# FudanCVL/SynFMC

Hardware: AMD Instinct MI355X
Metric: denoising steps/sec, 16x320x512 bf16 U-Net+CMC+OMC (higher is better)
Workload: dtype bf16; 1 GPU; 16x320x512 clip, CFG batch 2, full-width 3D U-Net (1.39B params, random init) + Camera Adapter (CMC) + Object Motion Control (OMC) features, DDIM step; configs/obj.yaml shapes; 1 clip per GPU; frames=16, height=320, width=512, hip_graph=True, fp8_temporal_attention=False, parallelism=dp1 (independent clips, no collective)

## Files before the change

include/fmc_hip.h:

```cpp
#ifndef FMC_HIP_H
#define FMC_HIP_H

#include <stdint.h>

#ifdef __cplusplus
extern "C" {
#endif

#define FMC_VERSION 100

enum { FMC_BF16 = 0, FMC_F32 = 1 };

enum {
    FMC_OK = 0,
    FMC_E_SHAPE = -1,
    FMC_E_DTYPE = -2,
    FMC_E_ALIGN = -3,
    FMC_E_LAUNCH = -4,
    FMC_E_NULL = -5
};

int fmc_version(void);
const char* fmc_last_error(void);

int64_t fmc_groupnorm_workspace_bytes(int N, int C, int G);
int fmc_groupnorm_silu_fwd(const void* x, void* y, const float* gamma, const float* beta, float* stats,
                           void* workspace, int N, int HW, int C, int G, float eps, int act, int dtype,
                           const void* x2, int C1, void* stream);
int fmc_groupnorm_silu_bwd(const void* dy, const void* x, void* dx, const float* gamma, const float* beta,
                           const float* stats, void* workspace, int N, int HW, int C, int G, int act,
                           int dtype, void* stream);

int fmc_layernorm_fwd(const void* x, void* y, const float* gamma, const float* beta, const float* pe,
                      int64_t M, int C, float eps, int pe_inner, int pe_frames, int dtype, void* stream);
int fmc_layernorm_add_fwd(const void* x, const void* addend, void* sum_out, void* y, const float* gamma, const float* beta,
                          const float* pe, int64_t M, int C, float eps, int pe_inner, int pe_frames, int dtype, void* stream);

int fmc_geglu_fwd(const void* x, void* y, int64_t M, int Cff, int dtype, void* stream);

int fmc_spatial_attn_fwd(const void* q, const void* k, const void* v, void* o, float* lse, int B, int H,
                         int Sq, int Skv, int D, int64_t q_batch_stride, int64_t q_row_stride,
                         int64_t kv_batch_stride, int64_t kv_row_stride, int64_t o_batch_stride,
                         int64_t o_row_stride, int kv_batch_div, float scale, int dtype, void* stream);

int fmc_temporal_attn_fwd(const void* q, const void* k, const void* v, void* o, int n_clips, int n_pix,
                          int F, int H, int D, int64_t clip_stride, int64_t frame_stride,
                          int64_t pix_stride, int64_t o_clip_stride, int64_t o_frame_stride,
                          int64_t o_pix_stride, float scale, int dtype, void* stream);

int fmc_plucker_fwd(const float* K, const float* c2w, void* out, int B, int F, int H, int W, int c2w_rows,
                    int layout, int dtype, void* stream);

int fmc_omc_rasterize_fwd(const float* poses, const float* masks, void* feat, float* mask_out, int BF,
                          int n_obj, int H, int W, int layout, int dtype, void* stream);

int fmc_gaussian_circle_mask_fwd(const float* circles, float* out, int N, int H, int W, void* stream);

int fmc_mask_modulate_fwd(const void* x, const float* mask_in, void* y, float* mask_out, int N, int h, int w,
                          int C, int Hin, int Win, int dtype, void* stream);

int fmc_feature_add_fwd(const void* h, const void* t, void* out, int64_t n_elems, int64_t skip_elems,
                        int dtype, void* stream);

int fmc_cfg_ddim_step(const void* eps_uc, const float* x, float* x_out, int64_t n, int has_uncond,
                      float guidance, float alpha_t, float alpha_prev, int dtype, void* stream);

typedef struct fmc_sampler_coef {
    float g;
    float m_x, m_e, m_clamp;
    float c_x, c_e, c_m, c_n;
    float c_h[3];
    float in_scale;
} fmc_sampler_coef;
int64_t fmc_sampler_step_elems_per_trip(void);
int fmc_sampler_step(const void* eps_uc, const float* x, const void* noise, const float* hist0, const float* hist1,
                     const float* hist2, float* x_out, float* m_out, void* x_in, int64_t n, int has_uncond, int n_hist,
                     int in_reps, fmc_sampler_coef coef, int dtype, int in_dtype, void* stream);

int fmc_linear_bf16(const void* x, const void* w, const void* bias, const void* residual, void* out, int64_t M, int N,
                    int K, int64_t ldx, int64_t ldres, int64_t ldo, float alpha, int epilogue, int tile, int split_k,
                    void* workspace, int64_t workspace_bytes, const void* x2, int64_t ldx2, int k_split,
                    const void* residual2, void* stream);

int fmc_conv3x3_bf16(const void* x, const void* w, const void* bias, const void* temb, const void* residual, void* out,
                     int n_img, int H, int W, int Cin, int Cout, int64_t temb_row_stride, int temb_img_div,
                     int upsample2x, int tile, int split_k, void* workspace, int64_t workspace_bytes, void* stream);

int fmc_linear_bf16_gn(const void* x, const void* w, const void* bias, const void* residual, void* out, int64_t M, int N, int K,
                       int64_t ldx, int64_t ldres, int64_t ldo, float alpha, const void* residual2, float* gn_partials, int gn_hw,
                       int w_tilemajor, void* stream);
int fmc_linear_bf16_ln(const void* x, const void* w, const void* bias, const void* residual, void* out, int64_t M, int N, int K,
                       int64_t ldx, int64_t ldres, int64_t ldo, float alpha, const void* residual2, void* ln_out, const float* ln_gamma,
                       const float* ln_beta, float ln_eps, const float* ln_pe, int ln_pe_inner, int ln_pe_frames, float* ln_stats, int w_tilemajor,
                       void* stream);
int fmc_linear_bf16_lnc(const void* x, const void* w_gamma, void* out, int64_t M, int N, int K, int64_t ldx, int64_t ldo, int epilogue,
                        const float* ln_stats, const float* ln_c, const float* ln_bias, int w_tilemajor, void* stream);
int fmc_linear_bf16_ffblk(const void* x, const void* w, const void* bias, const void* residual, void* out, int64_t M, int N, int K,
                          int64_t ldres, float alpha, int epilogue, int x_blocked, int out_blocked, const float* ln_stats, const float* ln_c,
                          const float* ln_bias, int w_tilemajor, void* stream);
int fmc_groupnorm_fold_linear(const float* partials, int part_splits, const float* gamma, const float* beta, const void* w, const void* bias,
                              void* w_out, float* bias_out, int n_img, int HW, int C, int G, int N, float eps, int w_tilemajor, void* stream);
int fmc_linear_bf16_imgw(const void* x, const void* w_img, const float* bias_img, void* out, int64_t M, int N, int K, int64_t ldx, int64_t ldo,
                         int img_rows, float* ln_stats, float ln_eps, int w_tilemajor, void* stream);
int fmc_linear_bf16_fftail(const void* x_blocked, const void* x2, const void* w, const void* bias, const void* residual, void* out, int64_t M,
                           int N, int K, int k_split, int64_t ldx2, int64_t ldres, float* gn_partials, int gn_hw, int w_tilemajor, void* stream);
int fmc_linear_bf16_ffblk_partial(const void* x_blocked, const void* w, const void* bias, const void* residual, void* out, int64_t M, int N, int K,
                                  int64_t ldres, float alpha, int w_tilemajor, void* stream);
int fmc_linear_bf16_fftail_partial(const void* x_blocked, const void* x2, const void* w, const void* bias, const void* residual, void* out, int64_t M,
                                   int N, int K, int k_split, int64_t ldx2, int64_t ldres, float* gn_partials, int gn_hw, int w_tilemajor, void* stream);
int fmc_conv3x3_bf16_gn(const void* x, const void* w, const void* bias, const void* temb, const void* residual, void* out, int n_img,
                        int H, int W, int Cin, int Cout, int64_t temb_row_stride, int temb_img_div, int upsample2x,
                        float* gn_partials, int w_tilemajor, void* stream);
int fmc_groupnorm_apply_fwd(const void* x, void* y, const float* gamma, const float* beta, float* stats, const float* partials,
                            int part_splits, int N, int HW, int C, int G, float eps, int act, int dtype, void* stream);

int fmc_linear4_supported(int64_t M, int N, int K, int64_t ldx);
int fmc_linear4_bf16(const void* x, const void* w, const void* bias, const void* residual, const void* residual2, void* out, int64_t M, int N, int K,
                     int64_t ldx, int64_t ldres, int64_t ldo, float alpha, void* stream);

int fmc_vendor_init(void);
int fmc_vendor_destroy(void);
int fmc_vendor_version(void);
int64_t fmc_vendor_workspace_bytes(void);
int fmc_vendor_linear_candidates(int64_t M, int N, int K, int64_t ldx, int64_t ldres, int64_t ldo, int has_bias, int has_residual);
int fmc_vendor_linear_bf16(const void* x, const void* w, const void* bias, const void* residual, void* out, int64_t M, int N, int K,
                           int64_t ldx, int64_t ldres, int64_t ldo, int algo, void* workspace, int64_t workspace_bytes, void* stream);

int fmc_attention_supported(int D);
int fmc_attention_fwd(const void* q, const void* k, const void* v, void* o, const unsigned char* key_keep, int B, int H, int Sq, int Skv, int D,
                      int64_t q_batch_stride, int64_t q_row_stride, int64_t kv_batch_stride, int64_t kv_row_stride, int64_t o_batch_stride,
                      int64_t o_row_stride, float scale, int causal, int dtype, void* stream);

int fmc_geglu_pipe_supported(int64_t M, int cff, int C, int variant);
int fmc_geglu_pipe_ln_bf16(const void* h, void* out, const float* ln_gamma, const float* ln_beta, float ln_eps, const void* w_packed, const void* bias,
                           int64_t M, int cff, int C, int out_blocked, int variant, void* stream);
int fmc_geglu_pipe_partial_supported(int64_t M, int cff, int C, int variant);
int fmc_geglu_pipe_ln_partial_bf16(const void* h, void* out, const float* ln_gamma, const float* ln_beta, float ln_eps, const void* w_packed, const void* bias,
                                   int64_t M, int cff, int C, int out_blocked, int variant, void* stream);

int fmc_groupnorm_partial_splits(int HW, int C);
int fmc_groupnorm_partials(const void* x, const void* x2, int C1, float* partials, int N, int HW, int C, int G, int dtype, void* stream);
int fmc_conv3x3_halo_supported(int n_img, int H, int W, int Cin, int Cin1, int Cout, int upsample2x);
int64_t fmc_conv3x3_halo_packed_bytes(int Cin, int Cout);
int fmc_conv3x3_halo_pack_weight(const void* w, void* dst, int Cin, int Cout, void* stream);
int fmc_conv3x3_halo_tiles_per_image(int H, int W);
int fmc_conv3x3_halo_bf16(const void* x, const void* x2, int Cin1, const void* w_packed, const void* bias, const void* temb, const void* residual,
                          void* out, int n_img, int H, int W, int Cin, int Cout, int64_t temb_row_stride, int temb_img_div, int upsample2x,
                          const float* gn_coef, int gn_act, float* gn_partials, void* stream);
int fmc_conv3x3_halo_sc_supported(int n_img, int H, int W, int Cin, int Cout, int Cin_sc, int Cin_sc1);
int64_t fmc_conv3x3_halo_sc_packed_bytes(int Cin, int Cout, int Cin_sc);
int64_t fmc_conv3x3_halo_sc_pack_source(int64_t chunk, int Cin, int Cin_sc, int tile_channels, int* from_shortcut);
int fmc_conv3x3_halo_sc_pack_weight(const void* w, const void* w_sc, void* dst, int Cin, int Cout, int Cin_sc, int tile_channels, void* stream);
int fmc_conv3x3_halo_sc_bf16(const void* x, const void* w_packed, const void* bias, const void* temb, void* out, const void* xs, const void* xs2,
                             int Cin_sc1, int Cin_sc, int n_img, int H, int W, int Cin, int Cout, int64_t temb_row_stride, int temb_img_div,
                             float* gn_partials, void* stream);
int fmc_conv3x3_halo4_supported(int n_img, int H, int W, int Cin, int Cin1, int Cout, int upsample2x, int wide);
int fmc_conv3x3_halo4_pack_weight(const void* w, void* dst, int Cin, int Cout, int wide, void* stream);
int fmc_conv3x3_halo4_row_blocks_per_image(int H, int W);
int fmc_conv3x3_halo4_tiles(int n_img, int H, int W, int Cout, int wide);
int fmc_conv3x3_halo4_bf16(const void* x, const void* x2, int Cin1, const void* w_packed, const void* bias, const void* temb, const void* residual,
                           void* out, int n_img, int H, int W, int Cin, int Cout, int64_t temb_row_stride, int temb_img_div, int upsample2x,
                           float* gn_partials, int split_k, void* workspace, int64_t workspace_bytes, int wide, void* stream);
int64_t fmc_conv3x3_upfold_packed_bytes(int Cin, int Cout);
int fmc_conv3x3_upfold_pack_weight(const void* w, void* dst, int Cin, int Cout, int tile_channels, void* stream);
int fmc_conv3x3_halo_fold_supported(int n_img, int Hs, int Ws, int Cin, int Cout);
int fmc_conv3x3_halo_fold_bf16(const void* x, const void* w_folded, const void* bias, void* out, int n_img, int Hs, int Ws, int Cin, int Cout,
                               float* gn_partials, void* stream);
int fmc_conv3x3_halo4_fold_supported(int n_img, int Hs, int Ws, int Cin, int Cout, int wide);
int fmc_conv3x3_halo4_fold_bf16(const void* x, const void* w_folded, const void* bias, void* out, int n_img, int Hs, int Ws, int Cin, int Cout,
                                float* gn_partials, int wide, void* stream);
int fmc_conv3x3_halo_partial_supported(int n_img, int H, int W, int Cin, int Cin1, int Cout, int upsample2x);
int fmc_conv3x3_halo_partial_tiles_per_image(int H, int W);
int fmc_conv3x3_halo_partial_bf16(const void* x, const void* x2, int Cin1, const void* w_packed, const void* bias, const void* temb,
                                  const void* residual, void* out, int n_img, int H, int W, int Cin, int Cout, int64_t temb_row_stride,
                                  int temb_img_div, int upsample2x, const float* gn_coef, int gn_act, float* gn_partials, void* stream);
int fmc_conv3x3_halo_sc_partial_supported(int n_img, int H, int W, int Cin, int Cout, int Cin_sc, int Cin_sc1);
int fmc_conv3x3_halo_sc_partial_bf16(const void* x, const void* w_packed, const void* bias, const void* temb, void* out, const void* xs,
                                     const void* xs2, int Cin_sc1, int Cin_sc, int n_img, int H, int W, int Cin, int Cout, int64_t temb_row_stride,
                                     int temb_img_div, float* gn_partials, void* stream);
int fmc_conv3x3_halo_fold_partial_supported(int n_img, int Hs, int Ws, int Cin, int Cout);
int fmc_conv3x3_halo_fold_partial_bf16(const void* x, const void* w_folded, const void* bias, void* out, int n_img, int Hs, int Ws, int Cin,
                                       int Cout, float* gn_partials, void* stream);
int fmc_conv3x3_halo4_partial_supported(int n_img, int H, int W, int Cin, int Cin1, int Cout, int upsample2x, int wide);
int fmc_conv3x3_halo4_partial_tw(int H, int W, int wide);
int fmc_conv3x3_halo4_partial_row_blocks_per_image(int H, int W, int tw);
int fmc_conv3x3_halo4_partial_tiles(int n_img, int H, int W, int Cout, int wide, int tw);
int fmc_conv3x3_halo4_partial_bf16(const void* x, const void* x2, int Cin1, const void* w_packed, const void* bias, const void* temb,
                                   const void* residual, void* out, int n_img, int H, int W, int Cin, int Cout, int64_t temb_row_stride,
                                   int temb_img_div, int upsample2x, float* gn_partials, int split_k, void* workspace, int64_t workspace_bytes,
                                   int wide, int tw, void* stream);
int fmc_conv3x3_halo4_fold_partial_supported(int n_img, int Hs, int Ws, int Cin, int Cout, int wide);
int fmc_conv3x3_halo4_fold_partial_bf16(const void* x, const void* w_folded, const void* bias, void* out, int n_img, int Hs, int Ws, int Cin,
                                        int Cout, float* gn_partials, int wide, int tw, void* stream);
int fmc_conv3x3_down_bwd_supported(int n_img, int H, int W, int Cin, int Cout);
int64_t fmc_conv3x3_down_bwd_packed_bytes(int Cin, int Cout);
int fmc_conv3x3_down_bwd_pack_weight(const void* w, void* dst, int Cin, int Cout, void* stream);
int fmc_conv3x3_down_bwd_tile(int n_img, int H, int W, int Cin, int Cout);
int fmc_conv3x3_down_bwd_bf16(const void* dy, const void* w_packed, void* dx, int n_img, int H, int W, int Cin, int Cout, int tile, void* stream);
int fmc_conv3x3_up_bwd_supported(int n_img, int Hs, int Ws, int Cin, int Cout);
int64_t fmc_conv3x3_up_bwd_packed_bytes(int Cin, int Cout);
int fmc_conv3x3_up_bwd_pack_weight(const void* w, void* dst, int Cin, int Cout, void* stream);
int fmc_conv3x3_up_bwd_tile(int n_img, int Hs, int Ws, int Cin, int Cout);
int fmc_conv3x3_up_bwd_bf16(const void* dy, const void* w_packed, void* dx, int n_img, int Hs, int Ws, int Cin, int Cout, int tile, void* stream);
int fmc_groupnorm_coef(const float* partials, int part_splits, const float* gamma, const float* beta, float* coef, float* stats, int N, int HW,
                       int C, int G, float eps, void* stream);

int fmc_split_bf16x3(const float* src, void* dst, int64_t rows, int C, int64_t ld_src, int64_t ld_dst, int col0, int K,
                     int role, void* stream);
int fmc_linear_x3_f32(const void* x3, const void* w3, const float* bias, const float* residual, float* out, int64_t M, int N,
                      int K3, int64_t ldx, int64_t ldres, int64_t ldo, float alpha, int epilogue, int tile, int split_k,
                      void* workspace, int64_t workspace_bytes, const float* residual2, void* stream);
int fmc_conv3x3_x3_f32(const void* x3, const void* w3, const float* bias, const float* temb, const float* residual, float* out,
                       int n_img, int H, int W, int Cin3, int Cout, int64_t temb_row_stride, int temb_img_div,
                       int upsample2x, int tile, int split_k, void* workspace, int64_t workspace_bytes, void* stream);

int fmc_layernorm_bwd(const void* dy, const void* x, const float* gamma, void* dx, float* dgamma, float* dbeta,
                      int64_t M, int C, float eps, int dtype, void* stream);
int fmc_layernorm_bwd_add(const void* dy, const void* x, const float* gamma, void* dx, float* dgamma, float* dbeta, const void* addend,
                          int64_t M, int C, float eps, int dtype, void* stream);
int fmc_groupnorm_silu_bwd_add(const void* dy, const void* x, void* dx, const float* gamma, const float* beta, const float* stats,
                               void* workspace, int N, int HW, int C, int G, int act, const void* addend, int dtype, void* stream);
int64_t fmc_groupnorm_silu_bwd_params_workspace_bytes(int N, int HW, int C, int G);
int fmc_groupnorm_silu_bwd_params(const void* dy, const void* x, void* dx, float* dgamma, float* dbeta, const float* gamma,
                                  const float* beta, const float* stats, const void* addend, int accumulate, void* workspace,
                                  int N, int HW, int C, int G, int act, int dtype, void* stream);
int64_t fmc_column_sum_workspace_bytes(int64_t M, int N);
int fmc_column_sum(const void* x, float* out, int64_t M, int N, int64_t ld, float alpha, int accumulate, void* workspace, int dtype,
                   void* stream);
int fmc_geglu_bwd(const void* dy, const void* x, void* dx, int64_t M, int Cff, int dtype, void* stream);
int fmc_spatial_attn_bwd(const void* q, const void* k, const void* v, const void* o, const void* d_o, const float* lse,
                         float* dvec, void* dq, void* dk, void* dv, int B, int H, int Sq, int Skv, int D,
                         int64_t q_batch_stride, int64_t q_row_stride, int64_t kv_batch_stride, int64_t kv_row_stride,
                         int64_t o_batch_stride, int64_t o_row_stride, int64_t dq_batch_stride, int64_t dq_row_stride,
                         int64_t dkv_batch_stride, int64_t dkv_row_stride, int kv_batch_div, float scale, int dtype,
                         void* stream);
int fmc_temporal_attn_bwd(const void* q, const void* k, const void* v, const void* d_o, void* dq, void* dk, void* dv,
                          int n_clips, int n_pix, int F, int H, int D, int64_t clip_stride, int64_t frame_stride,
                          int64_t pix_stride, int64_t do_clip_stride, int64_t do_frame_stride, int64_t do_pix_stride,
                          int64_t dq_clip_stride, int64_t dq_frame_stride, int64_t dq_pix_stride, float scale,
                          int dtype, void* stream);

int fmc_fp8_scales_roll(void* amax, void* scale, void* inv_scale, float margin, void* stream);
int fmc_linear_fp8_qkv(const void* x, const void* w, void* out_fp8, int64_t M, int N, int K, int64_t ldx,
                       const void* inv_scales, void* amax_bits, void* stream);
int fmc_temporal_attn_fp8_fwd(const void* q, const void* k, const void* v, void* o, const void* scales, int n_clips,
                              int n_pix, int F, int H, int D, int64_t clip_stride, int64_t frame_stride,
                              int64_t pix_stride, int64_t o_clip_stride, int64_t o_frame_stride, int64_t o_pix_stride,
                              float scale, void* stream);
int fmc_temporal_attn_fp8_bwd(const void* q, const void* k, const void* v, const void* scales, const void* d_o, void* dq,
                              void* dk, void* dv, int n_clips, int n_pix, int F, int H, int D, int64_t clip_stride,
                              int64_t frame_stride, int64_t pix_stride, int64_t do_clip_stride, int64_t do_frame_stride,
                              int64_t do_pix_stride, int64_t dq_clip_stride, int64_t dq_frame_stride,
                              int64_t dq_pix_stride, float scale, void* stream);

int fmc_nhwc_to_cmajor_padded(const void* src, void* dst, int n_img, int H, int W, int C, int64_t row_len, int guard,
                              int shifts, void* stream);
// ... 96 lines not shown
```

synfmc_amd/_lib.py:

```python
from __future__ import annotations

import ctypes
import os
from ctypes import c_char_p, c_float, c_int, c_int64, c_void_p

_HERE = os.path.dirname(os.path.abspath(__file__))
LIB_PATH = os.environ.get("FMC_HIP_LIB") or os.path.join(_HERE, "lib", "libfmc_hip.so")

FMC_BF16, FMC_F32 = 0, 1

_ERRORS = {-1: ValueError, -2: TypeError, -3: ValueError, -4: RuntimeError, -5: ValueError}


class SamplerCoef(ctypes.Structure):
    _fields_ = [("g", c_float), ("m_x", c_float), ("m_e", c_float), ("m_clamp", c_float), ("c_x", c_float), ("c_e", c_float),
                ("c_m", c_float), ("c_n", c_float), ("c_h", c_float * 3), ("in_scale", c_float)]

SIGNATURES = {
    "fmc_version": (c_int, []),
    "fmc_last_error": (c_char_p, []),
    "fmc_groupnorm_workspace_bytes": (c_int64, [c_int, c_int, c_int]),
    "fmc_groupnorm_silu_fwd": (c_int, [c_void_p, c_void_p, c_void_p, c_void_p, c_void_p, c_void_p, c_int, c_int, c_int,
                                       c_int, c_float, c_int, c_int, c_void_p, c_int, c_void_p]),
    "fmc_groupnorm_silu_bwd": (c_int, [c_void_p, c_void_p, c_void_p, c_void_p, c_void_p, c_void_p, c_void_p, c_int,
                                       c_int, c_int, c_int, c_int, c_int, c_void_p]),
    "fmc_layernorm_add_fwd": (c_int, [c_void_p, c_void_p, c_void_p, c_void_p, c_void_p, c_void_p, c_void_p, c_int64, c_int, c_float, c_int,
                                      c_int, c_int, c_void_p]),
    "fmc_layernorm_fwd": (c_int, [c_void_p, c_void_p, c_void_p, c_void_p, c_void_p, c_int64, c_int, c_float, c_int,
                                  c_int, c_int, c_void_p]),
    "fmc_geglu_fwd": (c_int, [c_void_p, c_void_p, c_int64, c_int, c_int, c_void_p]),
    "fmc_spatial_attn_fwd": (c_int, [c_void_p, c_void_p, c_void_p, c_void_p, c_void_p, c_int, c_int, c_int, c_int, c_int,
                                     c_int64, c_int64, c_int64, c_int64, c_int64, c_int64, c_int, c_float, c_int,
                                     c_void_p]),
    "fmc_temporal_attn_fwd": (c_int, [c_void_p, c_void_p, c_void_p, c_void_p, c_int, c_int, c_int, c_int, c_int,
                                      c_int64, c_int64, c_int64, c_int64, c_int64, c_int64, c_float, c_int, c_void_p]),
    "fmc_plucker_fwd": (c_int, [c_void_p, c_void_p, c_void_p, c_int, c_int, c_int, c_int, c_int, c_int, c_int, c_void_p]),
    "fmc_omc_rasterize_fwd": (c_int, [c_void_p, c_void_p, c_void_p, c_void_p, c_int, c_int, c_int, c_int, c_int, c_int,
                                      c_void_p]),
    "fmc_gaussian_circle_mask_fwd": (c_int, [c_void_p, c_void_p, c_int, c_int, c_int, c_void_p]),
    "fmc_mask_modulate_fwd": (c_int, [c_void_p, c_void_p, c_void_p, c_void_p, c_int, c_int, c_int, c_int, c_int, c_int,
                                      c_int, c_void_p]),
    "fmc_feature_add_fwd": (c_int, [c_void_p, c_void_p, c_void_p, c_int64, c_int64, c_int, c_void_p]),
    "fmc_cfg_ddim_step": (c_int, [c_void_p, c_void_p, c_void_p, c_int64, c_int, c_float, c_float, c_float, c_int,
                                  c_void_p]),
    "fmc_sampler_step_elems_per_trip": (c_int64, []),
    "fmc_sampler_step": (c_int, [c_void_p] * 9 + [c_int64, c_int, c_int, c_int, SamplerCoef, c_int, c_int, c_void_p]),
    "fmc_linear_bf16": (c_int, [c_void_p, c_void_p, c_void_p, c_void_p, c_void_p, c_int64, c_int, c_int, c_int64,
                                c_int64, c_int64, c_float, c_int, c_int, c_int, c_void_p, c_int64, c_void_p, c_int64, c_int,
                                c_void_p, c_void_p]),
    "fmc_linear_bf16_gn": (c_int, [c_void_p, c_void_p, c_void_p, c_void_p, c_void_p, c_int64, c_int, c_int, c_int64, c_int64, c_int64,
                                   c_float, c_void_p, c_void_p, c_int, c_int, c_void_p]),
    "fmc_linear_bf16_ln": (c_int, [c_void_p, c_void_p, c_void_p, c_void_p, c_void_p, c_int64, c_int, c_int, c_int64, c_int64, c_int64,
                                   c_float, c_void_p, c_void_p, c_void_p, c_void_p, c_float, c_void_p, c_int, c_int, c_void_p, c_int, c_void_p]),
    "fmc_linear_bf16_lnc": (c_int, [c_void_p, c_void_p, c_void_p, c_int64, c_int, c_int, c_int64, c_int64, c_int, c_void_p, c_void_p, c_void_p,
                                    c_int, c_void_p]),
    "fmc_linear_bf16_ffblk": (c_int, [c_void_p, c_void_p, c_void_p, c_void_p, c_void_p, c_int64, c_int, c_int, c_int64, c_float, c_int, c_int, c_int,
                                      c_void_p, c_void_p, c_void_p, c_int, c_void_p]),
    "fmc_groupnorm_fold_linear": (c_int, [c_void_p, c_int, c_void_p, c_void_p, c_void_p, c_void_p, c_void_p, c_void_p, c_int, c_int, c_int, c_int, c_int,
                                          c_float, c_int, c_void_p]),
    "fmc_linear_bf16_imgw": (c_int, [c_void_p, c_void_p, c_void_p, c_void_p, c_int64, c_int, c_int, c_int64, c_int64, c_int, c_void_p, c_float, c_int,
                                     c_void_p]),
    "fmc_linear_bf16_fftail": (c_int, [c_void_p, c_void_p, c_void_p, c_void_p, c_void_p, c_void_p, c_int64, c_int, c_int, c_int, c_int64, c_int64,
                                       c_void_p, c_int, c_int, c_void_p]),
    "fmc_conv3x3_bf16_gn": (c_int, [c_void_p, c_void_p, c_void_p, c_void_p, c_void_p, c_void_p, c_int, c_int, c_int, c_int, c_int,
                                    c_int64, c_int, c_int, c_void_p, c_int, c_void_p]),
    "fmc_groupnorm_partial_splits": (c_int, [c_int, c_int]),
    "fmc_groupnorm_partials": (c_int, [c_void_p, c_void_p, c_int, c_void_p, c_int, c_int, c_int, c_int, c_int, c_void_p]),
    "fmc_conv3x3_halo_supported": (c_int, [c_int, c_int, c_int, c_int, c_int, c_int, c_int]),
    "fmc_conv3x3_halo_packed_bytes": (c_int64, [c_int, c_int]),
    "fmc_conv3x3_halo_pack_weight": (c_int, [c_void_p, c_void_p, c_int, c_int, c_void_p]),
    "fmc_conv3x3_halo_tiles_per_image": (c_int, [c_int, c_int]),
    "fmc_conv3x3_halo_sc_supported": (c_int, [c_int, c_int, c_int, c_int, c_int, c_int, c_int]),
    "fmc_conv3x3_halo_sc_packed_bytes": (c_int64, [c_int, c_int, c_int]),
    "fmc_conv3x3_halo_sc_pack_source": (c_int64, [c_int64, c_int, c_int, c_int, ctypes.POINTER(c_int)]),
    "fmc_conv3x3_halo_sc_pack_weight": (c_int, [c_void_p, c_void_p, c_void_p, c_int, c_int, c_int, c_int, c_void_p]),
    "fmc_conv3x3_halo_sc_bf16": (c_int, [c_void_p, c_void_p, c_void_p, c_void_p, c_void_p, c_void_p, c_void_p, c_int, c_int, c_int, c_int, c_int,
                                         c_int, c_int, c_int64, c_int, c_void_p, c_void_p]),
    "fmc_conv3x3_halo_bf16": (c_int, [c_void_p, c_void_p, c_int, c_void_p, c_void_p, c_void_p, c_void_p, c_void_p, c_int, c_int, c_int, c_int, c_int,
                                      c_int64, c_int, c_int, c_void_p, c_int, c_void_p, c_void_p]),
    "fmc_conv3x3_halo4_supported": (c_int, [c_int, c_int, c_int, c_int, c_int, c_int, c_int, c_int]),
    "fmc_conv3x3_halo4_pack_weight": (c_int, [c_void_p, c_void_p, c_int, c_int, c_int, c_void_p]),
    "fmc_conv3x3_halo4_row_blocks_per_image": (c_int, [c_int, c_int]),
    "fmc_conv3x3_halo4_tiles": (c_int, [c_int, c_int, c_int, c_int, c_int]),
    "fmc_conv3x3_halo4_bf16": (c_int, [c_void_p, c_void_p, c_int, c_void_p, c_void_p, c_void_p, c_void_p, c_void_p, c_int, c_int, c_int, c_int, c_int,
                                       c_int64, c_int, c_int, c_void_p, c_int, c_void_p, c_int64, c_int, c_void_p]),
    "fmc_conv3x3_upfold_packed_bytes": (c_int64, [c_int, c_int]),
    "fmc_conv3x3_upfold_pack_weight": (c_int, [c_void_p, c_void_p, c_int, c_int, c_int, c_void_p]),
    "fmc_conv3x3_halo_fold_supported": (c_int, [c_int, c_int, c_int, c_int, c_int]),
    "fmc_conv3x3_halo_fold_bf16": (c_int, [c_void_p, c_void_p, c_void_p, c_void_p, c_int, c_int, c_int, c_int, c_int, c_void_p, c_void_p]),
    "fmc_conv3x3_halo4_fold_supported": (c_int, [c_int, c_int, c_int, c_int, c_int, c_int]),
    "fmc_conv3x3_halo4_fold_bf16": (c_int, [c_void_p, c_void_p, c_void_p, c_void_p, c_int, c_int, c_int, c_int, c_int, c_void_p, c_int, c_void_p]),
    "fmc_conv3x3_halo_partial_supported": (c_int, [c_int, c_int, c_int, c_int, c_int, c_int, c_int]),
    "fmc_conv3x3_halo_partial_tiles_per_image": (c_int, [c_int, c_int]),
    "fmc_conv3x3_halo_partial_bf16": (c_int, [c_void_p, c_void_p, c_int, c_void_p, c_void_p, c_void_p, c_void_p, c_void_p, c_int, c_int, c_int, c_int,
                                              c_int, c_int64, c_int, c_int, c_void_p, c_int, c_void_p, c_void_p]),
    "fmc_conv3x3_halo_sc_partial_supported": (c_int, [c_int, c_int, c_int, c_int, c_int, c_int, c_int]),
    "fmc_conv3x3_halo_sc_partial_bf16": (c_int, [c_void_p, c_void_p, c_void_p, c_void_p, c_void_p, c_void_p, c_void_p, c_int, c_int, c_int, c_int,
                                                 c_int, c_int, c_int, c_int64, c_int, c_void_p, c_void_p]),
    "fmc_conv3x3_halo_fold_partial_supported": (c_int, [c_int, c_int, c_int, c_int, c_int]),
    "fmc_conv3x3_halo_fold_partial_bf16": (c_int, [c_void_p, c_void_p, c_void_p, c_void_p, c_int, c_int, c_int, c_int, c_int, c_void_p, c_void_p]),
    "fmc_conv3x3_halo4_partial_supported": (c_int, [c_int, c_int, c_int, c_int, c_int, c_int, c_int, c_int]),
    "fmc_conv3x3_halo4_partial_tw": (c_int, [c_int, c_int, c_int]),
    "fmc_conv3x3_halo4_partial_row_blocks_per_image": (c_int, [c_int, c_int, c_int]),
    "fmc_conv3x3_halo4_partial_tiles": (c_int, [c_int, c_int, c_int, c_int, c_int, c_int]),
    "fmc_conv3x3_halo4_partial_bf16": (c_int, [c_void_p, c_void_p, c_int, c_void_p, c_void_p, c_void_p, c_void_p, c_void_p, c_int, c_int, c_int, c_int,
                                               c_int, c_int64, c_int, c_int, c_void_p, c_int, c_void_p, c_int64, c_int, c_int, c_void_p]),
    "fmc_conv3x3_halo4_fold_partial_supported": (c_int, [c_int, c_int, c_int, c_int, c_int, c_int]),
    "fmc_conv3x3_halo4_fold_partial_bf16": (c_int, [c_void_p, c_void_p, c_void_p, c_void_p, c_int, c_int, c_int, c_int, c_int, c_void_p, c_int, c_int,
                                                    c_void_p]),
    "fmc_conv3x3_down_bwd_supported": (c_int, [c_int, c_int, c_int, c_int, c_int]),
    "fmc_conv3x3_down_bwd_packed_bytes": (c_int64, [c_int, c_int]),
    "fmc_conv3x3_down_bwd_pack_weight": (c_int, [c_void_p, c_void_p, c_int, c_int, c_void_p]),
    "fmc_conv3x3_down_bwd_tile": (c_int, [c_int, c_int, c_int, c_int, c_int]),
    "fmc_conv3x3_down_bwd_bf16": (c_int, [c_void_p, c_void_p, c_void_p, c_int, c_int, c_int, c_int, c_int, c_int, c_void_p]),
    "fmc_conv3x3_up_bwd_supported": (c_int, [c_int, c_int, c_int, c_int, c_int]),
    "fmc_conv3x3_up_bwd_packed_bytes": (c_int64, [c_int, c_int]),
    "fmc_conv3x3_up_bwd_pack_weight": (c_int, [c_void_p, c_void_p, c_int, c_int, c_void_p]),
    "fmc_conv3x3_up_bwd_tile": (c_int, [c_int, c_int, c_int, c_int, c_int]),
    "fmc_conv3x3_up_bwd_bf16": (c_int, [c_void_p, c_void_p, c_void_p, c_int, c_int, c_int, c_int, c_int, c_int, c_void_p]),
    "fmc_linear4_supported": (c_int, [c_int64, c_int, c_int, c_int64]),
    "fmc_vendor_linear_candidates": (c_int, [c_int64, c_int, c_int, c_int64, c_int64, c_int64, c_int, c_int]),
    "fmc_vendor_linear_bf16": (c_int, [c_void_p, c_void_p, c_void_p, c_void_p, c_void_p, c_int64, c_int, c_int, c_int64, c_int64, c_int64, c_int, c_void_p,
                                       c_int64, c_void_p]),
    "fmc_geglu_pipe_supported": (c_int, [c_int64, c_int, c_int, c_int]),
    "fmc_geglu_pipe_ln_bf16": (c_int, [c_void_p, c_void_p, c_void_p, c_void_p, c_float, c_void_p, c_void_p, c_int64, c_int, c_int, c_int, c_int, c_void_p]),
    "fmc_geglu_pipe_partial_supported": (c_int, [c_int64, c_int, c_int, c_int]),
    "fmc_geglu_pipe_ln_partial_bf16": (c_int, [c_void_p, c_void_p, c_void_p, c_void_p, c_float, c_void_p, c_void_p, c_int64, c_int, c_int, c_int, c_int,
                                               c_void_p]),
    "fmc_linear_bf16_ffblk_partial": (c_int, [c_void_p, c_void_p, c_void_p, c_void_p, c_void_p, c_int64, c_int, c_int, c_int64, c_float, c_int, c_void_p]),
    "fmc_linear_bf16_fftail_partial": (c_int, [c_void_p, c_void_p, c_void_p, c_void_p, c_void_p, c_void_p, c_int64, c_int, c_int, c_int, c_int64, c_int64,
                                               c_void_p, c_int, c_int, c_void_p]),
    "fmc_attention_supported": (c_int, [c_int]),
    "fmc_attention_fwd": (c_int, [c_void_p, c_void_p, c_void_p, c_void_p, c_void_p, c_int, c_int, c_int, c_int, c_int, c_int64, c_int64, c_int64, c_int64,
                                  c_int64, c_int64, c_float, c_int, c_int, c_void_p]),
    "fmc_vendor_init": (c_int, []),
    "fmc_vendor_destroy": (c_int, []),
    "fmc_vendor_version": (c_int, []),
    "fmc_vendor_workspace_bytes": (c_int64, []),
    "fmc_linear4_bf16": (c_int, [c_void_p, c_void_p, c_void_p, c_void_p, c_void_p, c_void_p, c_int64, c_int, c_int, c_int64, c_int64, c_int64, c_float, c_void_p]),
    "fmc_groupnorm_coef": (c_int, [c_void_p, c_int, c_void_p, c_void_p, c_void_p, c_void_p, c_int, c_int, c_int, c_int, c_float, c_void_p]),
    "fmc_groupnorm_apply_fwd": (c_int, [c_void_p, c_void_p, c_void_p, c_void_p, c_void_p, c_void_p, c_int, c_int, c_int, c_int, c_int,
                                        c_float, c_int, c_int, c_void_p]),
    "fmc_split_bf16x3": (c_int, [c_void_p, c_void_p, c_int64, c_int, c_int64, c_int64, c_int, c_int, c_int, c_void_p]),
    "fmc_linear_x3_f32": (c_int, [c_void_p, c_void_p, c_void_p, c_void_p, c_void_p, c_int64, c_int, c_int, c_int64,
                                  c_int64, c_int64, c_float, c_int, c_int, c_int, c_void_p, c_int64, c_void_p, c_void_p]),
    "fmc_conv3x3_x3_f32": (c_int, [c_void_p, c_void_p, c_void_p, c_void_p, c_void_p, c_void_p, c_int, c_int, c_int,
                                   c_int, c_int, c_int64, c_int, c_int, c_int, c_int, c_void_p, c_int64, c_void_p]),
    "fmc_layernorm_bwd": (c_int, [c_void_p, c_void_p, c_void_p, c_void_p, c_void_p, c_void_p, c_int64, c_int, c_float,
                                  c_int, c_void_p]),
    "fmc_layernorm_bwd_add": (c_int, [c_void_p, c_void_p, c_void_p, c_void_p, c_void_p, c_void_p, c_void_p, c_int64, c_int, c_float,
                                      c_int, c_void_p]),
    "fmc_groupnorm_silu_bwd_add": (c_int, [c_void_p, c_void_p, c_void_p, c_void_p, c_void_p, c_void_p, c_void_p, c_int, c_int, c_int, c_int,
                                           c_int, c_void_p, c_int, c_void_p]),
    "fmc_groupnorm_silu_bwd_params_workspace_bytes": (c_int64, [c_int, c_int, c_int, c_int]),
    "fmc_groupnorm_silu_bwd_params": (c_int, [c_void_p] * 9 + [c_int, c_void_p] + [c_int] * 6 + [c_void_p]),
    "fmc_column_sum_workspace_bytes": (c_int64, [c_int64, c_int]),
    "fmc_column_sum": (c_int, [c_void_p, c_void_p, c_int64, c_int, c_int64, c_float, c_int, c_void_p, c_int, c_void_p]),
    "fmc_geglu_bwd": (c_int, [c_void_p, c_void_p, c_void_p, c_int64, c_int, c_int, c_void_p]),
    "fmc_spatial_attn_bwd": (c_int, [c_void_p] * 10 + [c_int] * 5 + [c_int64] * 10 + [c_int, c_float, c_int, c_void_p]),
    "fmc_temporal_attn_bwd": (c_int, [c_void_p] * 7 + [c_int] * 5 + [c_int64] * 9 + [c_float, c_int, c_void_p]),
    "fmc_fp8_scales_roll": (c_int, [c_void_p, c_void_p, c_void_p, c_float, c_void_p]),
    "fmc_linear_fp8_qkv": (c_int, [c_void_p, c_void_p, c_void_p, c_int64, c_int, c_int, c_int64, c_void_p, c_void_p, c_void_p]),
    "fmc_temporal_attn_fp8_fwd": (c_int, [c_void_p] * 5 + [c_int] * 5 + [c_int64] * 6 + [c_float, c_void_p]),
    "fmc_temporal_attn_fp8_bwd": (c_int, [c_void_p] * 8 + [c_int] * 5 + [c_int64] * 9 + [c_float, c_void_p]),
    "fmc_nhwc_to_cmajor_padded": (c_int, [c_void_p, c_void_p, c_int, c_int, c_int, c_int, c_int64, c_int, c_int, c_void_p]),
    "fmc_linear_wgrad_workspace_bytes": (c_int64, [c_void_p, c_int]),
    "fmc_linear_wgrad_bf16": (c_int, [c_void_p, c_int, c_void_p, c_int64, c_void_p]),
    "fmc_conv3x3_wgrad_supported": (c_int, [c_int, c_int, c_int, c_int, c_int, c_int]),
    "fmc_conv3x3_wgrad_workspace_bytes": (c_int64, [c_int, c_int, c_int, c_int, c_int, c_int]),
    "fmc_conv3x3_wgrad_bf16": (c_int, [c_void_p, c_void_p, c_void_p, c_int, c_int, c_int, c_int, c_int, c_int, c_int, c_float, c_int, c_void_p,
                               c_int64, c_void_p]),
    "fmc_optim_chunk_elems": (c_int, []),
    "fmc_optim_workspace_bytes": (c_int64, [c_int, c_int, c_int]),
    "fmc_optim_check_tables": (c_int, [c_void_p, c_int, c_void_p, c_int, c_int, c_int]),
    "fmc_optim_grad_norm": (c_int, [c_void_p, c_int, c_void_p, c_int, c_void_p, c_int, c_int, c_void_p, c_int64, c_void_p]),
    "fmc_optim_adamw_step": (c_int, [c_void_p, c_int, c_void_p, c_int, c_void_p, c_int, c_int, c_void_p, c_int64, c_void_p]),
    "fmc_avgpool2x2_fwd": (c_int, [c_void_p, c_void_p, c_int, c_int, c_int, c_int, c_void_p]),
    "fmc_avgpool2x2_bwd": (c_int, [c_void_p, c_void_p, c_int, c_int, c_int, c_int, c_void_p]),
    "fmc_relu_fwd": (c_int, [c_void_p, c_void_p, c_int64, c_void_p]),
    "fmc_relu_bwd": (c_int, [c_void_p, c_void_p, c_void_p, c_int64, c_void_p]),
    "fmc_add_bf16": (c_int, [c_void_p, c_void_p, c_void_p, c_int64, c_void_p]),
    "fmc_temporal_block_bf16": (c_int, [c_void_p, c_void_p, c_void_p, c_void_p, c_float, c_void_p, c_void_p, c_float, c_void_p, c_void_p, c_void_p,
                                        c_void_p, c_float, c_int, c_int, c_int, c_int, c_int, c_float, c_void_p]),
    "fmc_temporal_block_set_debug": (c_int, [c_void_p]),
    "fmc_xattn_block640_bf16": (c_int, [c_void_p, c_void_p, c_void_p, c_void_p, c_float, c_void_p, c_void_p, c_void_p, c_void_p, c_int, c_int, c_int, c_int,
                                        c_float, c_void_p]),
    "fmc_xattn_pack_kv": (c_int, [c_void_p, c_void_p, c_int, c_int, c_int64, c_void_p]),
    "fmc_geglu320_ln_bf16": (c_int, [c_void_p, c_void_p, c_void_p, c_void_p, c_float, c_void_p, c_void_p, c_int64, c_int, c_int, c_void_p]),
    "fmc_geglu640_ln_bf16": (c_int, [c_void_p, c_void_p, c_void_p, c_void_p, c_float, c_void_p, c_void_p, c_int64, c_int, c_int, c_void_p]),
    "fmc_xattn_pack_kv40": (c_int, [c_void_p, c_void_p, c_int, c_int, c_int64, c_void_p]),
    "fmc_xattn_block320_bf16": (c_int, [c_void_p, c_void_p, c_void_p, c_void_p, c_float, c_void_p, c_void_p, c_void_p, c_void_p, c_void_p, c_float,
                                        c_int, c_int, c_int, c_int, c_float, c_void_p]),
    "fmc_temporal_block_partial_bf16": (c_int, [c_void_p, c_void_p, c_void_p, c_void_p, c_float, c_void_p, c_void_p, c_float, c_void_p, c_void_p, c_void_p,
                                                c_void_p, c_float, c_int, c_int, c_int, c_int, c_int, c_float, c_void_p]),
    "fmc_xattn_block640_partial_bf16": (c_int, [c_void_p, c_void_p, c_void_p, c_void_p, c_float, c_void_p, c_void_p, c_void_p, c_void_p, c_int, c_int, c_int,
                                                c_int, c_float, c_void_p]),
    "fmc_xattn_block320_partial_bf16": (c_int, [c_void_p, c_void_p, c_void_p, c_void_p, c_float, c_void_p, c_void_p, c_void_p, c_void_p, c_void_p, c_float,
                                                c_int, c_int, c_int, c_int, c_float, c_void_p]),
    "fmc_mxfp8_tile_rows": (c_int, []),
    "fmc_mxfp8_tile_cols": (c_int, []),
    "fmc_linear_mxfp8_supported": (c_int, [c_int64, c_int, c_int, c_int]),
    "fmc_mxfp8_pack_weight": (c_int, [c_void_p, c_void_p, c_void_p, c_int, c_int, c_int, c_void_p]),
    "fmc_layernorm_mxfp8_fwd": (c_int, [c_void_p, c_void_p, c_void_p, c_void_p, c_void_p, c_int64, c_int, c_int64, c_float, c_void_p]),
    "fmc_linear_mxfp8": (c_int, [c_void_p, c_void_p, c_void_p, c_void_p, c_void_p, c_void_p, c_void_p, c_void_p, c_int64, c_int, c_int, c_int64, c_int64,
                                 c_int, c_void_p]),
    "fmc_conv3x3_bf16": (c_int,[c_void_p, c_void_p, c_void_p, c_void_p, c_void_p, c_void_p, c_int, c_int, c_int,
                                 c_int, c_int, c_int64, c_int, c_int, c_int, c_int, c_void_p, c_int64, c_void_p]),
}

_lib = None


class FmcLibraryMissing(ImportError):
    pass
# ... 24 lines not shown
```

synfmc_amd/csrc/gemm_conv.hip:

```cpp
#include <stdlib.h>

#include <algorithm>
#include <type_traits>

#include "common.h"

namespace {

constexpr int BK_MAX = 64;

struct GemmParams {
    const bf16_t* a; const bf16_t* w; const bf16_t* bias; const bf16_t* temb; const bf16_t* res; bf16_t* out;
    const bf16_t* res2;
    int64_t M; int N, K;
    int64_t lda, ldres, ldo;
    int img_h, img_w, cin, hw;
    int64_t temb_ld; int temb_div;
    const bf16_t* a2; int64_t lda2; int ksplit;
    int ups;
    float alpha;
    int tiles_m, tiles_n;
    int regepi;
    int tap_outer;
    int group_m;
// ... 2096 lines not shown
    auto up4 = [](const bf16_t* p, float (&o)[4]) {
        const u32x2 w = *reinterpret_cast<const u32x2*>(p);
        o[0] = __uint_as_float(w[0] << 16); o[1] = __uint_as_float(w[0] & 0xffff0000u);
        o[2] = __uint_as_float(w[1] << 16); o[3] = __uint_as_float(w[1] & 0xffff0000u);
    };
    float o[4] = {v[0], v[1], v[2], v[3]}, a[4];
    if (P.bias) {
        up4(P.bias + n, a);
#pragma unroll
        for (int j = 0; j < 4; ++j) o[j] += a[j];
    }
#pragma unroll
    for (int j = 0; j < 4; ++j) o[j] *= P.alpha;
    if (MODE == 1 && P.temb) {
        up4(P.temb + ((m / P.hw) / P.temb_div) * P.temb_ld + n, a);
#pragma unroll
        for (int j = 0; j < 4; ++j) o[j] += a[j];
    }
    if (P.res) {
        up4(P.res + m * P.ldres + n, a);
#pragma unroll
        for (int j = 0; j < 4; ++j) o[j] += a[j];
        if (P.res2) {
            up4(P.res2 + m * P.ldres + n, a);
#pragma unroll
            for (int j = 0; j < 4; ++j) o[j] += a[j];
        }
    }
    *reinterpret_cast<u32x2*>(P.out + m * P.ldo + n) = u32x2{pack_bf2(o[0], o[1]), pack_bf2(o[2], o[3])};
}

template <int MODE, int EPI, int WM, int WN, int BK, int STAGES, int MI = 2>
void launch_gemm_g(GemmParams& P, hipStream_t st) {
    constexpr int BM = 32 * MI * WM, BN = 64 * WN;
    P.tiles_m = (int)((P.M + BM - 1) / BM);
    P.tiles_n = (P.N + BN - 1) / BN;
    P.tap_outer = conv_tap_outer();
    static const int regepi = fmc_env_int("FMC_GEMM_REGEPI", 1);
    P.regepi = regepi;
    size_t lds = (size_t)STAGES * (BM + BN) * BK * sizeof(bf16_t) + 1024;
    const size_t slab = (size_t)64 * (BN + 8) * sizeof(float);
    if (slab > lds) lds = slab;
    const size_t staged = (size_t)BM * ((EPI == 1 ? BN / 2 : BN) + 8) * sizeof(bf16_t);
    const size_t lds_plain = (P.split_k == 1 && (EPI == 1 || !P.res2) && staged > lds) ? staged : lds;
    unsigned grid = (unsigned)(P.tiles_m * P.tiles_n * P.split_k);
    constexpr int by_waves = 16 / (WM * WN) > 0 ? 16 / (WM * WN) : 1;
    const int by_lds = (int)(160 * 1024 / (P.sk ? lds : lds_plain));
    const int per_cu = by_lds < by_waves ? (by_lds < 1 ? 1 : by_lds) : by_waves;
    P.group_m = xcd_group_m(P, MODE == 0, 32.0 * per_cu, BN, BM);
    if (P.sk) {
        const int64_t iters = (int64_t)P.tiles_m * P.tiles_n * (P.K / BK);
        const int g = (fmc_cu_count() * per_cu) & ~7;
        const int64_t need = (int64_t)g * BM * BN * (int64_t)sizeof(float) + 4096;
        if (STAGES != 2 || MI != 2 || g < 8 || iters < 4 * (int64_t)g || P.sk_ws_bytes < need || g * (int)sizeof(int) > 4096) {
            P.sk = 0;
        } else {
            P.sk = g;
            grid = (unsigned)g;
        }
    }
    if constexpr (STAGES == 2 && MI == 2) {
        if (P.sk) {
            fmc_launch<gemm_kernel<MODE, EPI, WM, WN, MI, BK, STAGES, true>>(dim3(grid), dim3(64 * WM * WN), lds, st, P);
            return;
        }
    }
    fmc_launch<gemm_kernel<MODE, EPI, WM, WN, MI, BK, STAGES, false>>(dim3(grid), dim3(64 * WM * WN), lds_plain, st, P);
    if (P.split_k > 1) {
        const int64_t chunks = P.M * (P.N / 8);
        hipLaunchKernelGGL(splitk_reduce_kernel, dim3((unsigned)((chunks + 255) / 256)), dim3(256), 0, st, P);
    }
}

template <int MODE, int EPI, int PF>
void launch_gemm8(GemmParams& P, hipStream_t st) {
    P.tiles_m = (int)((P.M + 255) / 256);
    P.tiles_n = (P.N + 255) / 256;
    P.tap_outer = conv_tap_outer();
    P.group_m = xcd_group_m(P, MODE == 0, 32.0, 1, 1);
    constexpr size_t ring = (size_t)2 * 512 * 64 * sizeof(bf16_t) + 1024;
    constexpr size_t staged = (size_t)256 * ((EPI != 0 ? 128 : 256) + 8) * sizeof(bf16_t);
    constexpr size_t lds = staged > ring ? staged : ring;
    constexpr auto plain = gemm8_kernel<MODE, EPI, PF, 0>, sk_main = gemm8_kernel<MODE, EPI, PF, 1>, sk_finish = gemm8_kernel<MODE, EPI, PF, 2>;
    const int tiles = P.tiles_m * P.tiles_n;
    P.sk_t0 = 0;
    if (P.sk && P.sk_hybrid && !P.sk_lock) {
        const int g = fmc_cu_count() & ~7;
        const int t0 = g >= 8 ? (tiles / g) * g : 0, rem = tiles - t0;
        const int64_t iters = (int64_t)rem * (P.K / 64);
        const int maxseg = (rem + g - 1) / (g > 0 ? g : 1) + 2;
        const int64_t need = (int64_t)g * maxseg * 256 * 256 * (int64_t)sizeof(float) + 4096;
        if (t0 > 0 && rem > 0 && iters >= 2 * (int64_t)g && P.sk_ws_bytes >= need && need < ((int64_t)1 << 31)) {
            P.sk = g;
            P.sk_maxseg = maxseg;
            P.sk_whole = 0;
            P.sk_t0 = t0;
            fmc_launch<sk_main>(dim3((unsigned)g), dim3(512), lds, st, P);
            fmc_launch<plain>(dim3((unsigned)t0), dim3(512), lds, st, P);
            fmc_launch<sk_finish>(dim3((unsigned)rem), dim3(512), lds, st, P);
            return;
        }
        if (rem == 0) P.sk = 0;
    }
    if (P.sk && P.sk_lock) {
        const int g = fmc_cu_count() & ~7, nkt = P.K / 64;
        int S = P.sk_lock > 1 ? P.sk_lock : 0;
        if (!S) {
            double best = 1e30;
            for (int s2 = 2; s2 <= 16 && s2 <= nkt / 4; ++s2) {
                const int L = (nkt + s2 - 1) / s2;
                if ((s2 - 1) * L >= nkt) continue;
                const int rounds = (tiles * s2 + g - 1) / (g > 0 ? g : 1);
                const double cost = rounds * (L * 1.9 + 4.0) + tiles * s2 * 0.06;
                if (cost < best) { best = cost; S = s2; }
            }
        }
        const int L = S ? (nkt + S - 1) / S : 0;
        const int64_t need = (int64_t)tiles * S * 256 * 256 * (int64_t)sizeof(float) + 4096;
        if (g >= 8 && S >= 2 && (S - 1) * L < nkt && P.sk_ws_bytes >= need && need < ((int64_t)1 << 31)) {
            P.sk = g;
            P.sk_lock = S;
            P.sk_lock_len = L;
            fmc_launch<sk_main>(dim3((unsigned)g), dim3(512), lds, st, P);
            if constexpr (EPI == 0) hipLaunchKernelGGL((sk_finish_kernel<MODE>), dim3((unsigned)tiles * 64), dim3(256), 0, st, P);
            else fmc_launch<sk_finish>(dim3((unsigned)tiles), dim3(512), lds, st, P);
            return;
        }
        P.sk_lock = 0;
    }
    if (P.sk) {
        const int64_t iters = (int64_t)tiles * (P.K / 64);
        const int g = fmc_cu_count() & ~7;
        const int maxseg = (tiles + g - 1) / g + 2;
        const int64_t need = (int64_t)g * maxseg * 256 * 256 * (int64_t)sizeof(float) + 4096;
        if (g >= 8 && iters >= 2 * (int64_t)g && P.sk_ws_bytes >= need && need < ((int64_t)1 << 31)) {
            P.sk = g;
            P.sk_maxseg = maxseg;
            P.sk_whole = 0;
            fmc_launch<sk_main>(dim3((unsigned)g), dim3(512), lds, st, P);
            fmc_launch<sk_finish>(dim3((unsigned)tiles), dim3(512), lds, st, P);
            return;
        }
        P.sk = 0;
    }
    fmc_launch<plain>(dim3((unsigned)tiles), dim3(512), lds, st, P);
}

constexpr int K320_K = 320;
template <int MI, int NI> constexpr int k320_stage_chunks() { return ((32 * MI * ((160 * NI + 8) / 8) + 63) / 64) * 64; }
template <int MI, int NI> constexpr size_t k320_lds() {
    return (size_t)2 * 32 * MI * K320_K * 2 + (size_t)k320_stage_chunks<MI, NI>() * 16 + 160 * NI * sizeof(float);
}

template <int MI, int NI, bool HAS_RES>
__global__ __launch_bounds__(320, (MI * NI == 1 ? 3 : (MI * NI == 2 ? 2 : 1))) void gemm_k320_kernel(const GemmParams P) {
    constexpr int K = K320_K, KS = K / 16, BM = 32 * MI, BN = 160 * NI, OP = BN + 8, CPR = K / 8, OCPR = OP / 8, WC = 32 * NI;
    constexpr int A_ELEMS = BM * K, A_PIECES = BM * CPR / 64, ST_PIECES = k320_stage_chunks<MI, NI>() / 64;
    constexpr int A_PPW = (A_PIECES + 4) / 5, ST_PPW = (ST_PIECES + 4) / 5;
    extern __shared__ __attribute__((aligned(16))) unsigned char smem_raw[];
    bf16_t* Abuf = reinterpret_cast<bf16_t*>(smem_raw);
    bf16_t* Os = Abuf + 2 * A_ELEMS;
    float* bias_s = reinterpret_cast<float*>(Os + k320_stage_chunks<MI, NI>() * 8);
    const int tid = threadIdx.x, lane = tid & 63, wave = __builtin_amdgcn_readfirstlane(tid >> 6);
    const int l31 = lane & 31, half = lane >> 5;
    const int n0 = blockIdx.y * BN;
    const int ntiles = (int)(P.M / BM);

    bf16x8 wf[KS][NI];
#pragma unroll
    for (int ni = 0; ni < NI; ++ni) {
        const bf16_t* wrow = P.w + (int64_t)(n0 + wave * WC + ni * 32 + l31) * K + half * 8;
#pragma unroll
        for (int ks = 0; ks < KS; ++ks) {
            union { bf16x8 v; u32x4 u; } t;
            t.u = *reinterpret_cast<const u32x4*>(wrow + ks * 16);
            wf[ks][ni] = t.v;
        }
    }
    for (int i = tid; i < BN; i += 320) bias_s[i] = P.bias ? bf2f(P.bias[n0 + i]) : 0.f;

    const __amdgpu_buffer_rsrc_t rsA = __builtin_amdgcn_make_buffer_rsrc((void*)P.a, 0, (int)(((P.M - 1) * P.lda + K) * 2), 0x00020000);
    const __amdgpu_buffer_rsrc_t rsR = __builtin_amdgcn_make_buffer_rsrc((void*)(HAS_RES ? P.res + n0 : P.a), 0,
                                                                         HAS_RES ? (int)(((P.M - 1) * P.ldres + BN) * 2) : 0, 0x00020000);
    constexpr unsigned OOB = 0x7ffffff0u;
    int lane_v = lane, tid_v = tid;
    auto a_vo = [&](int piece) {
        const int L = piece * 64 + lane_v, row = L / CPR, phys = L - row * CPR;
        return (unsigned)(row * (int)P.lda * 2 + (phys ^ ((row >> 1) & 7)) * 16);
    };
    auto r_vo = [&](int piece) {
        const int L = piece * 64 + lane_v, row = L / OCPR, cc = L - row * OCPR;
        return (row < BM && cc < BN / 8) ? (unsigned)(row * (int)P.ldres * 2 + cc * 16) : OOB;
    };
    auto dma = [&](const __amdgpu_buffer_rsrc_t& rs, unsigned voff, int soff, bf16_t* lds) {
        __builtin_amdgcn_raw_ptr_buffer_load_lds(rs, (__attribute__((address_space(3))) void*)lds, 16, (int)voff, soff, 0, 0);
    };
    auto load_a = [&](int tile, int buf) {
        const int soff = tile * BM * (int)P.lda * 2;
#pragma unroll
        for (int i = 0; i < A_PPW; ++i)
            if (wave + 5 * i < A_PIECES) dma(rsA, a_vo(wave + 5 * i), soff, Abuf + buf * A_ELEMS + (wave + 5 * i) * 512);
    };
    auto load_res = [&](int tile) {
        const int soff = tile * BM * (int)P.ldres * 2;
#pragma unroll
        for (int i = 0; i < ST_PPW; ++i)
            if (wave + 5 * i < ST_PIECES) dma(rsR, r_vo(wave + 5 * i), soff, Os + (wave + 5 * i) * 512);
    };

    const int sw = (l31 >> 1) & 7, x6 = sw & 6, b0 = half ^ (sw & 1);
    int dsel[4];
#pragma unroll
    for (int m = 0; m < 4; ++m) dsel[m] = l31 * K + (x6 - 2 * (x6 & (2 * m)) + b0) * 8;

    int t = blockIdx.x;
    if (t < ntiles) load_a(t, 0);
    if (t + (int)gridDim.x < ntiles) load_a(t + gridDim.x, 1);
    if (HAS_RES && t < ntiles) load_res(t);
    asm volatile("s_waitcnt vmcnt(0)" ::: "memory");
    __syncthreads();

    for (int it = 0; t < ntiles; t += gridDim.x, ++it) {
        const bf16_t* As = Abuf + (it & 1) * A_ELEMS;
        asm volatile("" : "+v"(lane_v), "+v"(tid_v));
        f32x16 acc[NI][MI];
#pragma unroll
        for (int a = 0; a < NI; ++a)
#pragma unroll
            for (int g = 0; g < 4; ++g) {
                const f32x4 bv = *reinterpret_cast<const f32x4*>(bias_s + wave * WC + a * 32 + 8 * g + 4 * half);
#pragma unroll
                for (int b = 0; b < MI; ++b)
#pragma unroll
                    for (int j = 0; j < 4; ++j) acc[a][b][4 * g + j] = bv[j];
            }
        bf16x8 af[2][MI];
        auto read_a = [&](int ks, bf16x8 (&f)[MI]) {
#pragma unroll
            for (int mi = 0; mi < MI; ++mi) {
                union { bf16x8 v; u32x4 u; } ta;
                ta.u = *reinterpret_cast<const u32x4*>(As + mi * 32 * K + dsel[ks & 3] + ks * 16);
                f[mi] = ta.v;
            }
        };
        read_a(0, af[0]);
#pragma unroll
        for (int ks = 0; ks < KS; ++ks) {
            if (ks + 1 < KS) read_a(ks + 1, af[(ks + 1) & 1]);
            __builtin_amdgcn_sched_barrier(0);
#pragma unroll
            for (int ni = 0; ni < NI; ++ni)
#pragma unroll
                for (int mi = 0; mi < MI; ++mi)
                    acc[ni][mi] = __builtin_amdgcn_mfma_f32_32x32x16_bf16(wf[ks][ni], af[ks & 1][mi], acc[ni][mi], 0, 0, 0);
            __builtin_amdgcn_sched_barrier(0);
        }
        asm volatile("s_waitcnt vmcnt(0) lgkmcnt(0)\n\ts_barrier" ::: "memory");
        asm volatile("" : "+v"(lane_v), "+v"(tid_v));
        const int l31_e = lane_v & 31, half_e = (lane_v >> 5) & 1;
        if (t + 2 * (int)gridDim.x < ntiles) load_a(t + 2 * gridDim.x, it & 1);

#pragma unroll
        for (int ni = 0; ni < NI; ++ni)
#pragma unroll
            for (int mi = 0; mi < MI; ++mi) {
                bf16_t* wbase = Os + (mi * 32 + l31_e) * OP + wave * WC + ni * 32 + 4 * half_e;
                u32x2 rw[4];
                if (HAS_RES) {
#pragma unroll
                    for (int g = 0; g < 4; ++g) rw[g] = *reinterpret_cast<const u32x2*>(wbase + 8 * g);
                }
#pragma unroll
                for (int g = 0; g < 4; ++g) {
                    float o[4];
#pragma unroll
                    for (int j = 0; j < 4; ++j) o[j] = P.alpha * acc[ni][mi][4 * g + j];
                    if (HAS_RES) {
                        o[0] += __uint_as_float(rw[g][0] << 16); o[1] += __uint_as_float(rw[g][0] & 0xffff0000u);
                        o[2] += __uint_as_float(rw[g][1] << 16); o[3] += __uint_as_float(rw[g][1] & 0xffff0000u);
                    }
                    *reinterpret_cast<u32x2*>(wbase + 8 * g) = u32x2{pack_bf2(o[0], o[1]), pack_bf2(o[2], o[3])};
                }
            }
        asm volatile("s_waitcnt lgkmcnt(0)\n\ts_barrier" ::: "memory");
        {
            bf16_t* og = P.out + (int64_t)t * BM * P.ldo + n0;
            for (int c = tid_v; c < BM * (BN / 8); c += 320) {
                const int r = c / (BN / 8), ch = c - r * (BN / 8);
                *reinterpret_cast<u32x4*>(og + (int64_t)r * P.ldo + ch * 8) = *reinterpret_cast<const u32x4*>(Os + r * OP + ch * 8);
            }
        }
        if (HAS_RES) {
            asm volatile("s_waitcnt lgkmcnt(0)\n\ts_barrier" ::: "memory");
            if (t + (int)gridDim.x < ntiles) load_res(t + gridDim.x);
        }
    }
}

inline int gemm_k320_cfg() {
    static const int v = fmc_env_int("FMC_K320_CFG", 22);
    return v;
}
bool gemm_k320_ok(const GemmParams& P) {
    const int bn = (gemm_k320_cfg() % 10 == 1) ? 160 : 320;
    return !P.f32io && P.hw <= 1 && P.K == K320_K && P.N % bn == 0 && P.M % 64 == 0 && !P.a2 && !P.res2 && P.split_k == 1 && !P.sk && !P.temb &&
           ((P.M - 1) * P.lda + P.K) * 2 < ((int64_t)1 << 31) && (!P.res || ((P.M - 1) * P.ldres + P.N) * 2 < ((int64_t)1 << 31));
}

template <int MI, int NI>
void launch_gemm_k320_c(GemmParams& P, hipStream_t st) {
    const size_t lds = k320_lds<MI, NI>();
    const int per_cu = MI * NI == 1 ? 3 : (MI * NI == 2 ? 2 : 1);
    const int tiles = (int)(P.M / (32 * MI)), slots = fmc_cu_count() * per_cu;
    dim3 grid((unsigned)(tiles < slots ? tiles : slots), (unsigned)(P.N / (160 * NI)));
    if (P.res) fmc_launch<gemm_k320_kernel<MI, NI, true>>(grid, dim3(320), lds, st, P);
    else fmc_launch<gemm_k320_kernel<MI, NI, false>>(grid, dim3(320), lds, st, P);
}
void launch_gemm_k320(GemmParams& P, hipStream_t st) {
    switch (gemm_k320_cfg()) {
        case 11: launch_gemm_k320_c<1, 1>(P, st); break;
        case 21: launch_gemm_k320_c<2, 1>(P, st); break;
        case 12: launch_gemm_k320_c<1, 2>(P, st); break;
        default: launch_gemm_k320_c<2, 2>(P, st); break;
    }
}

bool gemm160_ok(const GemmParams& P) {
    return P.N % 320 == 0 && !P.sk && (!P.a2 || P.a_blocked);
}
template <int MODE, int EPI>
void launch_gemm160(GemmParams& P, hipStream_t st) {
    P.tiles_m = (int)((P.M + 159) / 160);
    P.tiles_n = P.N / 320;
    P.tap_outer = 0;
    P.group_m = xcd_group_m(P, MODE == 0, 32.0, 320, 160);
    constexpr size_t lds = (size_t)5 * (160 + 320) * 32 * sizeof(bf16_t) + 1024;
    static_assert(lds >= (size_t)160 * 328 * 2 && lds >= (size_t)160 * 164 * 4, "epilogue staging fits the operand buffers");
    constexpr auto plain = gemm160_kernel<MODE, EPI>;
    if (P.split_k > 1) {
        if constexpr (EPI == 0) {
            fmc_launch<plain>(dim3((unsigned)(P.tiles_m * P.tiles_n * P.split_k)), dim3(512), lds, st, P);
            const int64_t chunks = P.M * (P.N / 8);
            hipLaunchKernelGGL(splitk_reduce_kernel, dim3((unsigned)((chunks + 255) / 256)), dim3(256), 0, st, P);
        }
        return;
    }
    if constexpr (MODE == 0) {
        const int persist = g160_persist();
        const int cus = fmc_cu_count() & ~7;
        if (persist && !P.f32io && P.M % 160 == 0 && ((persist == 2 || P.a_blocked || P.bias_img) ? P.tiles_m * P.tiles_n >= cus : P.tiles_m * P.tiles_n > cus) && cus >= 8) {
            constexpr size_t ldsp = (size_t)3 * (160 + 320) * 32 * sizeof(bf16_t) + 1024 + (EPI == 1 ? (size_t)160 * 168 * 2 + 4096 : (size_t)80 * 328 * 2 + 5120);
            const bool e0 = EPI == 0;
            const int form = e0 && P.bias_img ? (P.ln_stats ? 5 : 4) : e0 && P.a2 ? 6 : P.lnc_stats ? 1 : e0 && P.ln_out ? 2 : e0 && P.ln_stats ? 3 : 0;
            const dim3 grid((unsigned)cus), block(512);
            if (form == 0) fmc_launch<gemm160p_kernel<EPI, 5>>(grid, block, ldsp, st, P);
            else if (form == 1) fmc_launch<gemm160p_kernel<EPI, 5, 0, 1>>(grid, block, ldsp, st, P);
            if constexpr (EPI == 0) {
                if (form == 2) fmc_launch<gemm160p_kernel<0, 5, 1>>(grid, block, ldsp, st, P);
                else if (form == 3) fmc_launch<gemm160p_kernel<0, 5, 2>>(grid, block, ldsp, st, P);
                else if (form == 4) fmc_launch<gemm160p_kernel<0, 5, 0, 0, 0, 1>>(grid, block, ldsp, st, P);
                else if (form == 5) fmc_launch<gemm160p_kernel<0, 5, 2, 0, 0, 1>>(grid, block, ldsp, st, P);
                else if (form == 6) fmc_launch<gemm160p_kernel<0, 5, 0, 0, 1>>(grid, block, ldsp, st, P);
            }
            return;
        }
    }
    fmc_launch<plain>(dim3((unsigned)(P.tiles_m * P.tiles_n)), dim3(512), lds, st, P);
}

bool gemm256p_ok(const GemmParams& P) {
    const int cus = fmc_cu_count() & ~7;
    return P.N % 320 == 0 && P.M % 256 == 0 && !P.sk && !P.a2 && P.split_k == 1 && !P.f32io && cus >= 8 && (P.M / 256) * (P.N / 320) > cus;
}
void launch_gemm256p(GemmParams& P, hipStream_t st) {
    P.tiles_m = (int)(P.M / 256);
    P.tiles_n = P.N / 320;
    P.tap_outer = 0;
    P.group_m = xcd_group_m(P, true, 32.0, 320, 256);
    constexpr size_t ldsp = (size_t)3 * (256 + 320) * 32 * sizeof(bf16_t) + 1024 + (size_t)128 * 168 * 2;
    static_assert(ldsp <= 160 * 1024, "ring + staging fit the LDS");
    fmc_launch<gemm160p_kernel<1, 8>>(dim3((unsigned)(fmc_cu_count() & ~7)), dim3(512), ldsp, st, P);
}

bool gemm8_ok(GemmParams& P) {
    const int64_t a_elems = P.hw > 1 ? (P.ups == 1 ? (P.M / 4) * (int64_t)P.cin : P.M * (int64_t)P.cin * (P.ups == 2 ? 4 : 1))
                                     : (P.a2 && P.a_blocked ? P.M * (int64_t)P.ksplit : (P.M - 1) * P.lda + P.K);
    P.a_bytes = a_elems * 2;
    return P.split_k == 1 && (!P.a2 || P.a_blocked) && P.a_bytes < ((int64_t)1 << 31) && (int64_t)P.N * P.K * 2 < ((int64_t)1 << 31);
}

constexpr int GEMM_TILE_MAX = 22;

template <int MODE, int EPI>
void launch_gemm(GemmParams& P, int tile, hipStream_t st) {
    int g = gemm_geometry_override();
    if (g == 0) g = tile;
    if (g == 0) {
        auto tiles = [&](int bm, int bn) { return ((P.M + bm - 1) / bm) * ((P.N + bn - 1) / bn); };
        auto waste = [&](int bn) { return (double)(((P.N + bn - 1) / bn) * bn) / P.N; };
        if (tiles(256, 256) >= 256 && waste(256) <= 1.2) g = 3;
        else if (tiles(256, 128) >= 256 && waste(128) <= 1.25) g = 2;
        else g = 1;
    }
    if (g == 17) {
        if constexpr (MODE == 0 && EPI == 1) {
            if (gemm8_ok(P) && gemm256p_ok(P)) { launch_gemm256p(P, st); return; }
        }
        g = 16;
    }
    if (g == 16) {
        const int sk_keep = P.split_k;
        P.split_k = 1;
        const bool fits = gemm8_ok(P);
        P.split_k = sk_keep;
        if (fits && gemm160_ok(P)) { launch_gemm160<MODE, EPI>(P, st); return; }
        g = 13;
    }
    if ((g == 13 || g == 14) && !gemm8_ok(P)) g = 3;
    if (g == 15) {
        if constexpr (MODE == 0 && EPI == 0) {
            if (gemm_k320_ok(P)) { launch_gemm_k320(P, st); return; }
        }
        g = 5;
    }
    if constexpr (MODE == 0 && EPI == 0) {
        if (g >= 19 && g <= 22 && (P.split_k != 1 || P.res2 || P.sk || P.f32io)) g = 1;
        if (g == 19) { launch_gemm_g<0, 0, 2, 2, 64, 3, 1>(P, st); return; }
        if (g == 20) { launch_gemm_g<0, 0, 2, 2, 32, 4, 1>(P, st); return; }
        if (g == 21) { launch_gemm_g<0, 0, 4, 2, 64, 2, 1>(P, st); return; }
        if (g == 22) { launch_gemm_g<0, 0, 2, 4, 64, 2, 1>(P, st); return; }
    }
    switch (g) {
        case 14: launch_gemm8<MODE, EPI, 5>(P, st); break;
        case 13: launch_gemm8<MODE, EPI, 4>(P, st); break;
        case 12: launch_gemm_g<MODE, EPI, 2, 5, 32, 4>(P, st); break;
        case 11: launch_gemm_g<MODE, EPI, 2, 5, 64, 2>(P, st); break;
        case 10: launch_gemm_g<MODE, EPI, 4, 2, 32, 4>(P, st); break;
        case 9: launch_gemm_g<MODE, EPI, 2, 2, 32, 4>(P, st); break;
        case 8: launch_gemm_g<MODE, EPI, 4, 4, 32, 4>(P, st); break;
        case 7: launch_gemm_g<MODE, EPI, 4, 2, 64, 3>(P, st); break;
        case 6: launch_gemm_g<MODE, EPI, 4, 4, 32, 2>(P, st); break;
        case 5: launch_gemm_g<MODE, EPI, 4, 2, 32, 2>(P, st); break;
        case 4: launch_gemm_g<MODE, EPI, 2, 2, 32, 2>(P, st); break;
        case 3: launch_gemm_g<MODE, EPI, 4, 4, 64, 2>(P, st); break;
        case 2: launch_gemm_g<MODE, EPI, 4, 2, 64, 2>(P, st); break;
        default: launch_gemm_g<MODE, EPI, 2, 2, 64, 2>(P, st); break;
    }
}

int set_split_k(GemmParams& P, int split_k, void* workspace, int64_t workspace_bytes, bool plain_epilogue, const char* who) {
    P.split_k = 1;
    P.ws = nullptr;
    P.sk = 0;
    P.sk_t0 = 0;
    P.sk_flags = nullptr;
    P.sk_ws_bytes = 0;
    P.sk_hybrid = split_k == -2;
    P.sk_lock = split_k == -3 ? 1 : (split_k <= -16 ? -split_k - 16 : 0);
    P.sk_lock_len = 0;
    if (split_k <= -16 && (P.sk_lock < 2 || P.sk_lock > 64)) FMC_FAIL(FMC_E_SHAPE, "%s: split_k %d (k-lockstep chunks = -split_k - 16 in 2..64)", who, split_k);
    if (split_k == -1 || split_k == -2 || split_k == -3 || split_k <= -16) {
        if (!workspace || !fmc_aligned16(workspace) || workspace_bytes < 8192)
            FMC_FAIL(FMC_E_NULL, "%s: stream-K needs a 16-byte aligned, zero-initialised workspace", who);
        P.sk = 1;
        P.sk_flags = (int*)workspace;
        P.ws = (float*)((char*)workspace + 4096);
        P.sk_ws_bytes = workspace_bytes;
        return 0;
    }
    if (split_k <= 1) return 0;
    if (split_k > 16 || !plain_epilogue) FMC_FAIL(FMC_E_SHAPE, "%s: split_k %d (1..16, not with the GEGLU epilogue)", who, split_k);
    if (!workspace || !fmc_aligned16(workspace)) FMC_FAIL(FMC_E_NULL, "%s: split_k needs a 16-byte aligned workspace", who);
    if (workspace_bytes < (int64_t)split_k * P.M * P.N * (int64_t)sizeof(float))
        FMC_FAIL(FMC_E_SHAPE, "%s: workspace of %lld bytes < split_k*M*N*4", who, (long long)workspace_bytes);
    P.split_k = split_k;
    P.ws = (float*)workspace;
    return 0;
}

}

static int linear_impl(const void* x, const void* w, const void* bias, const void* residual, void* out, int64_t M,
                       int N, int K, int64_t ldx, int64_t ldres, int64_t ldo, float alpha, int epilogue, int tile,
                       int split_k, void* workspace, int64_t workspace_bytes, const void* x2, int64_t ldx2,
                       int k_split, const void* residual2, void* stream, int f32io, void* gn_partials = nullptr, int gn_hw = 0,
                       void* ln_out = nullptr, const float* ln_gamma = nullptr, const float* ln_beta = nullptr, float ln_eps = 0.f,
                       const float* ln_pe = nullptr, int ln_pe_inner = 1, int ln_pe_frames = 1, float* ln_stats = nullptr,
                       const float* lnc_stats = nullptr, const float* lnc_c = nullptr, const float* lnc_bias = nullptr, int a_blocked = 0,
                       int out_blocked = 0, int w_tilemajor = 0, const float* bias_img = nullptr, int img_rows = 0) {
    if (!x || !w || !out) FMC_FAIL(FMC_E_NULL, "linear_bf16: NULL tensor");
    if (tile == 18) { tile = 16; w_tilemajor = 1; }
    if (M <= 0 || N <= 0 || K <= 0 || K % BK_MAX || N % 8 || ldx % 8 || ldo % (f32io ? 4 : 8) || (residual && ldres % (f32io ? 4 : 8)))
        FMC_FAIL(FMC_E_SHAPE, "linear_bf16: need K%%64==0, N%%8==0 and strides %%8==0 (M=%lld N=%d K=%d)", (long long)M, N, K);
    if (f32io && (x2 || split_k < 0)) FMC_FAIL(FMC_E_SHAPE, "linear_x3_f32: no two-source operand (split it into one buffer) and no stream-K");
    if (epilogue != 0 && epilogue != 1) FMC_FAIL(FMC_E_SHAPE, "linear_bf16: epilogue %d", epilogue);
    if (epilogue == 1 && (N % 64 || residual)) FMC_FAIL(FMC_E_SHAPE, "linear_bf16: GEGLU needs N%%64==0 and no residual");
    if (!fmc_aligned16(x) || !fmc_aligned16(w) || !fmc_aligned16(out) || (residual && !fmc_aligned16(residual)) ||
        (bias && !fmc_aligned16(bias)))
        FMC_FAIL(FMC_E_ALIGN, "linear_bf16: tensors must be 16-byte aligned");
    GemmParams P{};
    P.a = (const bf16_t*)x; P.w = (const bf16_t*)w; P.bias = (const bf16_t*)bias; P.temb = nullptr;
    if (residual2 && (!residual || !fmc_aligned16(residual2)))
        FMC_FAIL(FMC_E_NULL, "linear_bf16: residual2 needs residual (same row stride) and 16-byte alignment");
    P.res = (const bf16_t*)residual; P.res2 = (const bf16_t*)residual2; P.out = (bf16_t*)out;
    P.M = M; P.N = N; P.K = K; P.lda = ldx; P.ldres = ldres; P.ldo = ldo;
    P.img_h = P.img_w = P.cin = 0; P.hw = 1; P.alpha = alpha; P.temb_ld = 0; P.temb_div = 1; P.ups = 0;
    P.f32io = f32io;
    if (gn_partials && (f32io || epilogue != 0 || tile != 16 || split_k != 1 || gn_hw <= 0 || gn_hw % 160 || M % gn_hw || N % 320 || (x2 && !a_blocked) ||
                        ((M - 1) * ldx + K) * 2 >= ((int64_t)1 << 31) || (int64_t)N * K * 2 >= ((int64_t)1 << 31)))
        FMC_FAIL(FMC_E_SHAPE, "linear_bf16: GroupNorm partials come out of tile 16's plain bf16 epilogue only (N %% 320 == 0, pixels per image %% 160 == 0)");
    P.gn_part = (float*)gn_partials; P.gn_hw = gn_hw;
    if (lnc_stats) {
        const int cus = fmc_cu_count() & ~7;
        if (f32io || tile != 16 || split_k != 1 || gn_partials || ln_out || ln_stats || x2 || bias || residual || residual2 || alpha != 1.f || N % 320 ||
            M % 160 || (M / 160) * (N / 320) <= cus || cus < 8 || !lnc_c || !lnc_bias || !fmc_aligned16(lnc_c) || !fmc_aligned16(lnc_bias) ||
            ((M - 1) * ldx + K) * 2 >= ((int64_t)1 << 31) || (int64_t)N * K * 2 >= ((int64_t)1 << 31) ||
            g160_persist() == 0)
            FMC_FAIL(FMC_E_SHAPE, "linear_bf16_lnc: tile 16's persistent form only (bf16, N %% 320 == 0, M %% 160 == 0, more tiles than CUs, no bf16 bias / "
                                  "residual, alpha 1)");
    }
    P.lnc_stats = lnc_stats; P.lnc_c = lnc_c; P.lnc_bias = lnc_bias;
    if (a_blocked || out_blocked) {
        const int cus = fmc_cu_count() & ~7;
        if (f32io || tile != 16 || split_k != 1 || (gn_partials && !(a_blocked && x2 && !out_blocked)) || (x2 && (!a_blocked || out_blocked)) || N % 320 || M % 160 || cus < 8 ||
            (out_blocked && (M / 160) * (N / 320) <= cus) ||
            (a_blocked && (M / 160) * (N / 320) < cus) ||
            (a_blocked && (epilogue != 0 || ldx != (x2 ? k_split : K) || K % 32)) ||
            (x2 && (ln_out || ln_stats || lnc_stats || ((M - 1) * ldx2 + (K - k_split)) * 2 >= ((int64_t)1 << 31))) || (out_blocked && (epilogue != 1 || ldo != N / 2 || (N / 2) % 32)) ||
            (int64_t)M * (a_blocked ? K : N / 2) * 2 >= ((int64_t)1 << 31) || g160_persist() == 0)
            FMC_FAIL(FMC_E_SHAPE, "linear_bf16: the tile-major feed-forward intermediate needs tile 16's persistent form (M %% 160 == 0, N %% 320 == 0, "
                                  "more tiles than CUs, dense rows)");
    }
    P.a_blocked = a_blocked; P.out_blocked = out_blocked;
    P.bias_img = nullptr; P.w_img_stride = 0; P.img_rows = 0;
    if (bias_img) {
        const int cus = fmc_cu_count() & ~7;
        if (f32io || epilogue != 0 || tile != 16 || split_k != 1 || gn_partials || x2 || bias || residual || residual2 || alpha != 1.f || ln_out || lnc_stats ||
            a_blocked || out_blocked || N % 320 || M % 160 || (M / 160) * (N / 320) < cus || cus < 8 || img_rows < 160 || img_rows % 160 || M % img_rows ||
            ((uintptr_t)bias_img & 15) || ((M - 1) * ldx + K) * 2 >= ((int64_t)1 << 31) || (M / img_rows) * (int64_t)N * K * 2 >= ((int64_t)1 << 31) ||
            g160_persist() == 0)
            FMC_FAIL(FMC_E_SHAPE, "linear_bf16_imgw: tile 16's persistent form only (bf16, N %% 320 == 0, M %% 160 == 0, at least as many tiles as CUs, images of a multiple "
                                  "of 160 rows, no bf16 bias / residual, all weights < 2 GiB)");
        P.bias_img = bias_img; P.w_img_stride = (int64_t)N * K; P.img_rows = img_rows;
    }
    if (ln_out || ln_stats) {
        const int cus = fmc_cu_count() & ~7;
        if ((ln_out != nullptr) == (ln_stats != nullptr)) FMC_FAIL(FMC_E_NULL, "linear_bf16_ln: exactly one of ln_out / ln_stats");
        if (f32io || epilogue != 0 || tile != 16 || split_k != 1 || gn_partials || x2 || N != 320 || M % 160 || (bias_img ? M / 160 < cus : M / 160 <= cus) || cus < 8 ||
            (ln_out && (!ln_gamma || !ln_beta || !fmc_aligned16(ln_out))) || (ln_stats && ((uintptr_t)ln_stats & 7)) || (ln_pe && (ln_pe_inner <= 0 || ln_pe_inner % 160 || ln_pe_frames <= 0)) ||
            ((M - 1) * ldx + K) * 2 >= ((int64_t)1 << 31) || g160_persist() == 0)
            FMC_FAIL(FMC_E_SHAPE, "linear_bf16_ln: the LayerNorm output comes out of tile 16's persistent form only (bf16, N == 320, M %% 160 == 0, "
                                  "M / 160 > CUs, plain epilogue, positional-encoding frames of a multiple of 160 rows)");
    }
    P.ln_stats = ln_stats;
    P.ln_out = (bf16_t*)ln_out; P.ln_gamma = ln_gamma; P.ln_beta = ln_beta; P.ln_eps = ln_eps; P.ln_pe = ln_pe;
    P.ln_pe_inner = ln_pe_inner; P.ln_pe_frames = ln_pe_frames;
    if (x2 && (k_split <= 0 || k_split >= K || k_split % BK_MAX || ldx2 % 8 || !fmc_aligned16(x2)))
        FMC_FAIL(FMC_E_SHAPE, "linear_bf16: two-source input needs 0 < k_split < K, k_split %% 64 == 0 (k_split=%d K=%d)", k_split, K);
    P.a2 = (const bf16_t*)x2; P.lda2 = ldx2; P.ksplit = x2 ? k_split : 0;
    hipStream_t st = (hipStream_t)stream;
    if (tile < 0 || tile > GEMM_TILE_MAX) FMC_FAIL(FMC_E_SHAPE, "linear_bf16: tile %d", tile);
    P.w_blocked = 0;
    if (w_tilemajor) {
        if (tile != 16 || f32io || N % 320 || (x2 && !a_blocked) || split_k < 1 || ((M - 1) * ldx + K) * 2 >= ((int64_t)1 << 31) || (int64_t)N * K * 2 >= ((int64_t)1 << 31))
            FMC_FAIL(FMC_E_SHAPE, "linear_bf16: a tile-major weight (tile 18) needs bf16, N %% 320 == 0, no two-source operand, no stream-K, operands < 2 GiB");
        P.w_blocked = 1;
    }
    if (int rc = set_split_k(P, split_k, workspace, workspace_bytes, epilogue == 0, "linear_bf16")) return rc;
    if (epilogue == 0) launch_gemm<0, 0>(P, tile, st); else launch_gemm<0, 1>(P, tile, st);
    FMC_CHECK_LAUNCH("fmc_linear_bf16");
    return 0;
}

extern "C" int fmc_linear_bf16(const void* x, const void* w, const void* bias, const void* residual, void* out, int64_t M,
                               int N, int K, int64_t ldx, int64_t ldres, int64_t ldo, float alpha, int epilogue, int tile,
                               int split_k, void* workspace, int64_t workspace_bytes, const void* x2, int64_t ldx2,
                               int k_split, const void* residual2, void* stream) {
    return linear_impl(x, w, bias, residual, out, M, N, K, ldx, ldres, ldo, alpha, epilogue, tile, split_k, workspace,
                       workspace_bytes, x2, ldx2, k_split, residual2, stream, 0);
}

extern "C" int fmc_linear_bf16_gn(const void* x, const void* w, const void* bias, const void* residual, void* out, int64_t M,
                                  int N, int K, int64_t ldx, int64_t ldres, int64_t ldo, float alpha, const void* residual2,
                                  float* gn_partials, int gn_hw, int w_tilemajor, void* stream) {
    if (!gn_partials) FMC_FAIL(FMC_E_NULL, "linear_bf16_gn: NULL gn_partials");
    return linear_impl(x, w, bias, residual, out, M, N, K, ldx, ldres, ldo, alpha, 0, 16, 1, nullptr, 0, nullptr, 0, 0, residual2, stream, 0,
                       gn_partials, gn_hw, nullptr, nullptr, nullptr, 0.f, nullptr, 1, 1, nullptr, nullptr, nullptr, nullptr, 0, 0, w_tilemajor);
}

extern "C" int fmc_linear_bf16_ln(const void* x, const void* w, const void* bias, const void* residual, void* out, int64_t M,
                                  int N, int K, int64_t ldx, int64_t ldres, int64_t ldo, float alpha, const void* residual2,
                                  void* ln_out, const float* ln_gamma, const float* ln_beta, float ln_eps, const float* ln_pe,
                                  int ln_pe_inner, int ln_pe_frames, float* ln_stats, int w_tilemajor, void* stream) {
    if (!ln_out && !ln_stats) FMC_FAIL(FMC_E_NULL, "linear_bf16_ln: NULL ln_out and ln_stats");
    if (ln_out && (!ln_gamma || !ln_beta)) FMC_FAIL(FMC_E_NULL, "linear_bf16_ln: NULL gamma / beta");
    return linear_impl(x, w, bias, residual, out, M, N, K, ldx, ldres, ldo, alpha, 0, 16, 1, nullptr, 0, nullptr, 0, 0, residual2, stream, 0,
                       nullptr, 0, ln_out, ln_gamma, ln_beta, ln_eps, ln_pe, ln_pe_inner, ln_pe_frames, ln_stats, nullptr, nullptr, nullptr, 0, 0, w_tilemajor);
}

extern "C" int fmc_linear_bf16_lnc(const void* x, const void* w_gamma, void* out, int64_t M, int N, int K, int64_t ldx, int64_t ldo, int epilogue,
                                   const float* ln_stats, const float* ln_c, const float* ln_bias, int w_tilemajor, void* stream) {
    if (!ln_stats || !ln_c || !ln_bias) FMC_FAIL(FMC_E_NULL, "linear_bf16_lnc: NULL ln_stats / ln_c / ln_bias");
    return linear_impl(x, w_gamma, nullptr, nullptr, out, M, N, K, ldx, 0, ldo, 1.f, epilogue, 16, 1, nullptr, 0, nullptr, 0, 0, nullptr, stream, 0,
                       nullptr, 0, nullptr, nullptr, nullptr, 0.f, nullptr, 1, 1, nullptr, ln_stats, ln_c, ln_bias, 0, 0, w_tilemajor);
}

extern "C" int fmc_linear_bf16_ffblk(const void* x, const void* w, const void* bias, const void* residual, void* out, int64_t M, int N, int K,
                                     int64_t ldres, float alpha, int epilogue, int x_blocked, int out_blocked, const float* ln_stats,
                                     const float* ln_c, const float* ln_bias, int w_tilemajor, void* stream) {
    if (!x_blocked && !out_blocked) FMC_FAIL(FMC_E_SHAPE, "linear_bf16_ffblk: neither operand is tile-major (use fmc_linear_bf16)");
    const int n_out = epilogue == 1 ? N / 2 : N;
    return linear_impl(x, w, bias, residual, out, M, N, K, K, ldres, n_out, alpha, epilogue, 16, 1, nullptr, 0, nullptr, 0, 0, nullptr, stream, 0,
                       nullptr, 0, nullptr, nullptr, nullptr, 0.f, nullptr, 1, 1, nullptr, ln_stats, ln_c, ln_bias, x_blocked, out_blocked, w_tilemajor);
}

extern "C" int fmc_linear_bf16_imgw(const void* x, const void* w_img, const float* bias_img, void* out, int64_t M, int N, int K, int64_t ldx, int64_t ldo,
                                    int img_rows, float* ln_stats, float ln_eps, int w_tilemajor, void* stream) {
    if (!bias_img) FMC_FAIL(FMC_E_NULL, "linear_bf16_imgw: NULL bias_img");
    return linear_impl(x, w_img, nullptr, nullptr, out, M, N, K, ldx, 0, ldo, 1.f, 0, 16, 1, nullptr, 0, nullptr, 0, 0, nullptr, stream, 0,
                       nullptr, 0, nullptr, nullptr, nullptr, ln_eps, nullptr, 1, 1, ln_stats, nullptr, nullptr, nullptr, 0, 0, w_tilemajor, bias_img, img_rows);
}

extern "C" int fmc_linear_bf16_fftail(const void* x_blocked, const void* x2, const void* w, const void* bias, const void* residual, void* out, int64_t M,
                                      int N, int K, int k_split, int64_t ldx2, int64_t ldres, float* gn_partials, int gn_hw, int w_tilemajor, void* stream) {
    if (!x2) FMC_FAIL(FMC_E_NULL, "linear_bf16_fftail: NULL x2 (use fmc_linear_bf16_ffblk)");
    return linear_impl(x_blocked, w, bias, residual, out, M, N, K, k_split, ldres, N, 1.f, 0, 16, 1, nullptr, 0, x2, ldx2, k_split, nullptr, stream, 0,
                       gn_partials, gn_hw, nullptr, nullptr, nullptr, 0.f, nullptr, 1, 1, nullptr, nullptr, nullptr, nullptr, 1, 0, w_tilemajor);
}

extern "C" int fmc_linear_x3_f32(const void* x3, const void* w3, const float* bias, const float* residual, float* out, int64_t M,
                                 int N, int K3, int64_t ldx, int64_t ldres, int64_t ldo, float alpha, int epilogue, int tile,
                                 int split_k, void* workspace, int64_t workspace_bytes, const float* residual2, void* stream) {
    if (K3 % 3 || (K3 / 3) % 8) FMC_FAIL(FMC_E_SHAPE, "linear_x3_f32: K3 = 3 K of the split operands (K3=%d)", K3);
    return linear_impl(x3, w3, bias, residual, out, M, N, K3, ldx, ldres, ldo, alpha, epilogue, tile, split_k, workspace,
                       workspace_bytes, nullptr, 0, 0, residual2, stream, 1);
}

static int conv3x3_impl(const void* x, const void* w, const void* bias, const void* temb, const void* residual,
                        void* out, int n_img, int H, int W, int Cin, int Cout, int64_t temb_row_stride,
                        int temb_img_div, int upsample2x, int tile, int split_k,
                        void* workspace, int64_t workspace_bytes, void* stream, int f32io, void* gn_partials = nullptr, int w_tilemajor = 0) {
    if (!x || !w || !out) FMC_FAIL(FMC_E_NULL, "conv3x3_bf16: NULL tensor");
    if (tile == 18) { tile = 16; w_tilemajor = 1; }
    if (n_img <= 0 || H <= 0 || W <= 0 || Cin <= 0 || Cout <= 0 || Cin % BK_MAX || Cout % 8)
        FMC_FAIL(FMC_E_SHAPE, "conv3x3_bf16: need Cin%%64==0 and Cout%%8==0 (Cin=%d Cout=%d)", Cin, Cout);
    if (!fmc_aligned16(x) || !fmc_aligned16(w) || !fmc_aligned16(out) || (residual && !fmc_aligned16(residual)) ||
        (temb && !fmc_aligned16(temb)) || (bias && !fmc_aligned16(bias)))
        FMC_FAIL(FMC_E_ALIGN, "conv3x3_bf16: tensors must be 16-byte aligned");
    GemmParams P{};
    P.a = (const bf16_t*)x; P.w = (const bf16_t*)w; P.bias = (const bf16_t*)bias; P.temb = (const bf16_t*)temb;
    P.res = (const bf16_t*)residual; P.res2 = nullptr; P.out = (bf16_t*)out;
    P.M = (int64_t)n_img * H * W; P.N = Cout; P.K = 9 * Cin; P.lda = Cin; P.ldres = Cout; P.ldo = Cout;
    P.a2 = nullptr; P.lda2 = 0; P.ksplit = 0;
    P.img_h = H; P.img_w = W; P.cin = Cin; P.hw = H * W; P.alpha = 1.f;
    if (temb && (temb_img_div < 1 || temb_row_stride % (f32io ? 4 : 8))) FMC_FAIL(FMC_E_SHAPE, "conv3x3_bf16: temb_img_div >= 1, temb_row_stride %% 8 == 0");
    P.f32io = f32io;
    if (gn_partials && (f32io || tile != 16 || split_k != 1 || (H * W) % 160 || Cout % 320 ||
                        (int64_t)n_img * H * W * Cin * 2 * (upsample2x == 2 ? 4 : 1) >= ((int64_t)1 << 31) || (int64_t)Cout * 9 * Cin * 2 >= ((int64_t)1 << 31)))
        FMC_FAIL(FMC_E_SHAPE, "conv3x3_bf16: GroupNorm partials come out of tile 16's plain bf16 epilogue only (Cout %% 320 == 0, H W %% 160 == 0)");
    P.gn_part = (float*)gn_partials; P.gn_hw = H * W;
    if (f32io && split_k < 0) FMC_FAIL(FMC_E_SHAPE, "conv3x3_x3_f32: no stream-K in fp32-storage mode");
    P.temb_ld = temb_row_stride; P.temb_div = temb_img_div < 1 ? 1 : temb_img_div;
    if (upsample2x < 0 || upsample2x > 2) FMC_FAIL(FMC_E_SHAPE, "conv3x3_bf16: resample mode %d", upsample2x);
    if (upsample2x == 1 && ((H | W) & 1)) FMC_FAIL(FMC_E_SHAPE, "conv3x3_bf16: upsample2x needs even H, W (the OUTPUT size)");
    P.ups = upsample2x;
    if (tile < 0 || tile > GEMM_TILE_MAX) FMC_FAIL(FMC_E_SHAPE, "conv3x3_bf16: tile %d", tile);
    P.w_blocked = 0;
    if (w_tilemajor) {
        if (tile != 16 || f32io || Cout % 320 || Cin % 64 || split_k < 1 || (int64_t)Cout * 9 * Cin * 2 >= ((int64_t)1 << 31) ||
            (int64_t)n_img * H * W * Cin * 2 * (upsample2x == 2 ? 4 : 1) >= ((int64_t)1 << 31))
            FMC_FAIL(FMC_E_SHAPE, "conv3x3_bf16: tile 18 (tile-major filter) needs bf16, Cout %% 320 == 0, Cin %% 64 == 0, no stream-K, operands < 2 GiB");
        P.w_blocked = 1;
    }
    if (int rc = set_split_k(P, split_k, workspace, workspace_bytes, true, "conv3x3_bf16")) return rc;
    launch_gemm<1, 0>(P, tile, (hipStream_t)stream);
    FMC_CHECK_LAUNCH("fmc_conv3x3_bf16");
    return 0;
}

extern "C" int fmc_conv3x3_bf16(const void* x, const void* w, const void* bias, const void* temb, const void* residual,
                                void* out, int n_img, int H, int W, int Cin, int Cout, int64_t temb_row_stride,
                                int temb_img_div, int upsample2x, int tile, int split_k,
                                void* workspace, int64_t workspace_bytes, void* stream) {
    return conv3x3_impl(x, w, bias, temb, residual, out, n_img, H, W, Cin, Cout, temb_row_stride, temb_img_div, upsample2x, tile,
                        split_k, workspace, workspace_bytes, stream, 0);
}

extern "C" int fmc_conv3x3_bf16_gn(const void* x, const void* w, const void* bias, const void* temb, const void* residual,
                                   void* out, int n_img, int H, int W, int Cin, int Cout, int64_t temb_row_stride,
                                   int temb_img_div, int upsample2x, float* gn_partials, int w_tilemajor, void* stream) {
    if (!gn_partials) FMC_FAIL(FMC_E_NULL, "conv3x3_bf16_gn: NULL gn_partials");
    return conv3x3_impl(x, w, bias, temb, residual, out, n_img, H, W, Cin, Cout, temb_row_stride, temb_img_div, upsample2x, 16, 1,
                        nullptr, 0, stream, 0, gn_partials, w_tilemajor);
}

extern "C" int fmc_conv3x3_x3_f32(const void* x3, const void* w3, const float* bias, const float* temb, const float* residual,
                                  float* out, int n_img, int H, int W, int Cin3, int Cout, int64_t temb_row_stride,
                                  int temb_img_div, int upsample2x, int tile, int split_k,
                                  void* workspace, int64_t workspace_bytes, void* stream) {
    if (Cin3 % 3) FMC_FAIL(FMC_E_SHAPE, "conv3x3_x3_f32: Cin3 = 3 Cin of the split operands (Cin3=%d)", Cin3);
    return conv3x3_impl(x3, w3, bias, temb, residual, out, n_img, H, W, Cin3, Cout, temb_row_stride, temb_img_div, upsample2x, tile,
                        split_k, workspace, workspace_bytes, stream, 1);
}

namespace {
__global__ __launch_bounds__(256) void split_bf16x3_kernel(const float* __restrict__ src, bf16_t* __restrict__ dst, int64_t rows, int C,
                                                           int64_t ld_src, int64_t ld_dst, int col0, int K, int role) {
    const int cpr = C / 8;
    const int64_t idx = (int64_t)blockIdx.x * 256 + threadIdx.x;
    if (idx >= rows * cpr) return;
    const int64_t r = idx / cpr;
    const int c = (int)(idx - r * cpr) * 8;
    float v[8];
    Vec8<float>::load(src + r * ld_src + c, v);
    bf16x8 hi, lo;
    split_bf16x8(v, hi, lo);
    union { bf16x8 v; u32x4 u; } h, l;
    h.v = hi; l.v = lo;
    bf16_t* d = dst + r * ld_dst + col0 + c;
    *reinterpret_cast<u32x4*>(d) = h.u;
    *reinterpret_cast<u32x4*>(d + K) = role == 0 ? h.u : l.u;
    *reinterpret_cast<u32x4*>(d + 2 * (int64_t)K) = role == 0 ? l.u : h.u;
}
}

extern "C" int fmc_split_bf16x3(const float* src, void* dst, int64_t rows, int C, int64_t ld_src, int64_t ld_dst, int col0, int K,
                                int role, void* stream) {
    if (!src || !dst) FMC_FAIL(FMC_E_NULL, "split_bf16x3: NULL tensor");
    if (rows <= 0 || C <= 0 || C % 8 || K % 8 || col0 % 8 || col0 < 0 || col0 + C > K || ld_src % 4 || ld_dst % 8 || ld_dst < 3 * (int64_t)K ||
        (role != 0 && role != 1))
        FMC_FAIL(FMC_E_SHAPE, "split_bf16x3: rows=%lld C=%d K=%d col0=%d ld_src=%lld ld_dst=%lld role=%d", (long long)rows, C, K, col0,
                 (long long)ld_src, (long long)ld_dst, role);
    if (!fmc_aligned16(src) || !fmc_aligned16(dst)) FMC_FAIL(FMC_E_ALIGN, "split_bf16x3: tensors must be 16-byte aligned");
    const int64_t chunks = rows * (C / 8);
    hipLaunchKernelGGL(split_bf16x3_kernel, dim3((unsigned)((chunks + 255) / 256)), dim3(256), 0, (hipStream_t)stream, src,
                       (bf16_t*)dst, rows, C, ld_src, ld_dst, col0, K, role);
    FMC_CHECK_LAUNCH("fmc_split_bf16x3");
    return 0;
}

extern "C" int fmc_linear_fp8_qkv(const void* x, const void* w, void* out_fp8, int64_t M, int N, int K, int64_t ldx,
                                  const void* inv_scales, void* amax_bits, void* stream) {
    if (!x || !w || !out_fp8 || !inv_scales) FMC_FAIL(FMC_E_NULL, "linear_fp8_qkv: NULL tensor");
    if (M <= 0 || N <= 0 || K <= 0 || K % BK_MAX || N % 192 || ldx % 8)
        FMC_FAIL(FMC_E_SHAPE, "linear_fp8_qkv: need K%%64==0, N = 3*C with C%%64==0, ldx%%8==0 (M=%lld N=%d K=%d)", (long long)M, N, K);
    if (!fmc_aligned16(x) || !fmc_aligned16(w) || !fmc_aligned16(out_fp8)) FMC_FAIL(FMC_E_ALIGN, "linear_fp8_qkv: tensors must be 16-byte aligned");
    GemmParams P{};
    P.a = (const bf16_t*)x; P.w = (const bf16_t*)w; P.out = (bf16_t*)out_fp8;
    P.M = M; P.N = N; P.K = K; P.lda = ldx; P.ldo = N / 2;
    P.hw = 1; P.alpha = 1.f; P.temb_div = 1; P.split_k = 1;
    P.q8_inv = (const float*)inv_scales; P.q8_amax = (unsigned*)amax_bits;
    if (!gemm8_ok(P)) FMC_FAIL(FMC_E_SHAPE, "linear_fp8_qkv: operands beyond 2 GiB");
    launch_gemm8<0, 2, 4>(P, (hipStream_t)stream);
    FMC_CHECK_LAUNCH("fmc_linear_fp8_qkv");
    return 0;
}

static int ff_partial_impl(const char* who, const void* xb, const void* x2, const void* w, const void* bias, const void* residual, void* out, int64_t M, int N,
                           int K, int k_split, int64_t ldx2, int64_t ldres, float alpha, int w_tilemajor, void* stream) {
    if (!xb || !w || !out) FMC_FAIL(FMC_E_NULL, "%s: NULL tensor", who);
    const int cus = fmc_cu_count() & ~7;
    const int64_t tiles_m = (M + 159) / 160, Mp = tiles_m * 160;
    const int ka = x2 ? k_split : K;
    if (M <= 0 || N <= 0 || K <= 0 || N % 320 || K % BK_MAX || cus < 8 || tiles_m * (N / 320) < cus || g160_persist() == 0 || (residual && ldres % 8) ||
        (x2 && (k_split <= 0 || k_split >= K || k_split % BK_MAX || ldx2 % 8 || ldx2 < K - k_split || ((M - 1) * ldx2 + (K - k_split)) * 2 >= ((int64_t)1 << 31))) ||
        Mp * (int64_t)ka * 2 >= ((int64_t)1 << 31) || (int64_t)N * K * 2 >= ((int64_t)1 << 31))
        FMC_FAIL(FMC_E_SHAPE, "%s: need N %% 320 == 0, K %% 64 == 0, ceil(M / 160) * (N / 320) >= CUs, operands below 2 GiB (M=%lld N=%d K=%d k_split=%d)", who,
                 (long long)M, N, K, k_split);
    if (!fmc_aligned16(xb) || !fmc_aligned16(w) || !fmc_aligned16(out) || (x2 && !fmc_aligned16(x2)) || (residual && !fmc_aligned16(residual)) ||
        (bias && !fmc_aligned16(bias)))
        FMC_FAIL(FMC_E_ALIGN, "%s: tensors must be 16-byte aligned", who);
    GemmParams P{};
    P.a = (const bf16_t*)xb; P.w = (const bf16_t*)w; P.bias = (const bf16_t*)bias; P.res = (const bf16_t*)residual; P.out = (bf16_t*)out;
    P.M = M; P.N = N; P.K = K; P.lda = ka; P.ldres = ldres; P.ldo = N; P.hw = 1; P.alpha = alpha; P.temb_div = 1;
// ... 31 lines not shown
```

synfmc_amd/hip_ops.py:

```python
from __future__ import annotations

import atexit
import ctypes
import math
import os
from typing import Optional, Tuple

import torch

from . import _lib
from ._lib import FMC_BF16, FMC_F32
from .derived import derived_on_owner

_DT = {torch.bfloat16: FMC_BF16, torch.float32: FMC_F32}


def _dt(t: torch.Tensor) -> int:
    try:
        return _DT[t.dtype]
    except KeyError:
        raise TypeError(f"fmc kernels take bf16 or fp32 activations, got {t.dtype}") from None


def _dev(*ts: torch.Tensor) -> None:
# ... 1475 lines not shown
        k_split = x.shape[-1]
        assert M2 == M and k_split + x2.shape[-1] == Kd
    n_out = N // 2 if geglu else N
    ldo = n_out
    if out is None:
        out = torch.empty(*x.shape[:-1], n_out, dtype=x.dtype, device=x.device)
    else:
        assert out.dtype == x.dtype and out.shape[-1] == n_out and _rows2d(out)[0] == M and tile != 18
        ldo = _rows2d(out)[1]
    ldres = 0
    if residual is not None:
        assert residual.shape == out.shape
        _, ldres = _rows2d(residual)
    if residual2 is not None:
        assert residual is not None and residual2.shape == out.shape and _rows2d(residual2)[1] == ldres
    ws, ws_bytes = _splitk_workspace(x.device, split_k, M, N)
    _log_call("own_linear", (M, N, Kd, "geglu" if geglu else f"t{tile}", (residual is not None) + (residual2 is not None)), 2.0 * M * N * Kd)
    _lib.check(_lib.load().fmc_linear_bf16(x.data_ptr(), weight.data_ptr(), _p(bias), _p(residual), out.data_ptr(), M, N,
                                           Kd, ldx, ldres, ldo, float(alpha), int(geglu), int(tile), int(split_k),
                                           ws, ws_bytes, _p(x2), ldx2, k_split, _p(residual2), _stream()),
               "fmc_linear_bf16")
    return out


def conv3x3_supported(x: torch.Tensor, weight: torch.Tensor, stride, padding) -> bool:
    s2 = tuple(stride) == (2, 2) and x.shape[-1] % 2 == 0 and x.shape[-2] % 2 == 0
    return (x.is_cuda and x.dtype == torch.bfloat16 and weight.dtype == torch.bfloat16
            and tuple(weight.shape[2:]) == (3, 3) and (tuple(stride) == (1, 1) or s2) and tuple(padding) == (1, 1)
            and weight.shape[1] % 64 == 0 and weight.shape[0] % 8 == 0)


def conv3x3_bf16(x_nhwc: torch.Tensor, weight_cl: torch.Tensor, bias: Optional[torch.Tensor] = None,
                 temb: Optional[torch.Tensor] = None, residual_nhwc: Optional[torch.Tensor] = None,
                 tile: int = 0, split_k: int = 1, temb_div: int = 1, upsample: bool = False,
                 stride2: bool = False) -> torch.Tensor:
    _dev(x_nhwc, weight_cl, bias, temb, residual_nhwc)
    n, h, w, cin = x_nhwc.shape
    if upsample:
        h, w = 2 * h, 2 * w
    if stride2:
        assert not upsample and h % 2 == 0 and w % 2 == 0
        h, w = h // 2, w // 2
    cout = weight_cl.shape[0]
    assert x_nhwc.is_contiguous() and weight_cl.is_contiguous(memory_format=torch.channels_last)
    assert temb is None or (temb.stride(1) == 1 and temb.shape == (n // temb_div, cout) and n % temb_div == 0)
    assert residual_nhwc is None or (residual_nhwc.is_contiguous() and residual_nhwc.shape == (n, h, w, cout))
    out = torch.empty(n, h, w, cout, dtype=x_nhwc.dtype, device=x_nhwc.device)
    tile, split_k = _decode_arm(tile, split_k)
    if tile == 18:
        if cout % 320 or cin % 64 or split_k < 1 or x_nhwc.numel() * 2 >= (1 << 31) or weight_cl.numel() * 2 >= (1 << 31):
            tile = 16
        else:
            weight_cl = _w_tilemajor_conv(weight_cl)
    ws, ws_bytes = _splitk_workspace(x_nhwc.device, split_k, n * h * w, cout)
    _lib.check(_lib.load().fmc_conv3x3_bf16(x_nhwc.data_ptr(), weight_cl.data_ptr(), _p(bias), _p(temb),
                                            _p(residual_nhwc), out.data_ptr(), n, h, w, cin, cout,
                                            0 if temb is None else temb.stride(0), int(temb_div), 2 if stride2 else int(upsample),
                                            int(tile),
                                            int(split_k), ws, ws_bytes, _stream()),
               "fmc_conv3x3_bf16")
    return out


LN_EPILOGUE = os.environ.get("FMC_LN_EPILOGUE", "1") != "0"
ln_epilogue_calls = {"emitted": 0, "consumed": 0}


class LnSpec:
    __slots__ = ("gamma", "beta", "eps", "pe", "pe_inner", "pe_frames", "key", "stats_only")

    def __init__(self, gamma, beta, eps, pe, pe_inner, pe_frames, key, stats_only: bool = False):
        self.gamma, self.beta, self.eps, self.pe, self.pe_inner, self.pe_frames, self.key = gamma, beta, eps, pe, pe_inner, pe_frames, key
        self.stats_only = stats_only


_cu_count = {}


def _cus(device) -> int:
    n = _cu_count.get(device.index)
    if n is None:
        n = _cu_count[device.index] = torch.cuda.get_device_properties(device).multi_processor_count & ~7
    return n


def ln_emit_ok(x: torch.Tensor, weight: torch.Tensor, residual, residual2, ln: LnSpec) -> bool:
    N, Kd = weight.shape
    M = x.numel() // x.shape[-1]
    return (LN_EPILOGUE and not torch.is_grad_enabled() and x.is_cuda and x.dtype == torch.bfloat16 and weight.dtype == torch.bfloat16
            and x.is_contiguous() and weight.is_contiguous() and N == 320 and Kd % 64 == 0 and M % 160 == 0 and M // 160 > _cus(x.device)
            and ln.gamma.numel() == 320 and ln.gamma.dtype == torch.float32 and ln.beta.dtype == torch.float32
            and (ln.pe is None or (ln.pe.dtype == torch.float32 and ln.pe.is_contiguous() and ln.pe.shape[-1] == 320 and ln.pe_inner % 160 == 0
                                   and ln.pe.shape[0] >= ln.pe_frames))
            and (residual is None or (residual.is_contiguous() and residual.dtype == x.dtype))
            and (residual2 is None or residual2.is_contiguous()) and M * max(Kd, 320) * 2 < (1 << 31) and os.environ.get("FMC_G160_PERSIST", "1") != "0")


def carry_ln(src: torch.Tensor, dst: torch.Tensor) -> torch.Tensor:
    tag = getattr(src, "_fmc_ln", None)
    if tag is not None:
        dst._fmc_ln = tag
    return dst


def take_ln(x: torch.Tensor, key) -> Optional[torch.Tensor]:
    tag = getattr(x, "_fmc_ln", None)
    if tag is None or tag[1] != key or torch.is_grad_enabled() or tag[2]:
        return None
    ln_epilogue_calls["consumed"] += 1
    return tag[0].view(x.shape)


def take_ln_stats(x: torch.Tensor, key) -> Optional[torch.Tensor]:
    tag = getattr(x, "_fmc_ln", None)
    if tag is None or tag[1] != key or torch.is_grad_enabled() or not tag[2]:
        return None
    return tag[0]


def pending_ln(x: torch.Tensor, stats: torch.Tensor, gamma: torch.Tensor, beta: torch.Tensor, eps: float) -> torch.Tensor:
    v = x.view(x.shape)
    v._fmc_pending_ln = (stats, gamma, beta, eps)
    return v


def resolve_pending_ln(x: torch.Tensor) -> torch.Tensor:
    pend = getattr(x, "_fmc_pending_ln", None)
    if pend is None:
        return x
    ln_epilogue_calls["materialised"] = ln_epilogue_calls.get("materialised", 0) + 1
    return _layernorm_raw(x.contiguous(), pend[1], pend[2], pend[3], None, 1, 1)


def _ln_folded_weight(weight: torch.Tensor, bias: Optional[torch.Tensor], gamma: torch.Tensor, beta: torch.Tensor):
    def build():
        w32 = weight.detach().float()
        wg = (w32 * gamma.float()[None, :]).to(torch.bfloat16).contiguous()
        b = w32 @ beta.float()
        if bias is not None:
            b = b + bias.detach().float()
        return wg, wg.float().sum(dim=1).contiguous(), b.contiguous()
    tag = (gamma.data_ptr(), gamma._version, beta.data_ptr(), beta._version, None if bias is None else (bias.data_ptr(), bias._version))
    return derived_on_owner(weight, "_fmc_lnw", tag, build)


def lnc_ok(x: torch.Tensor, weight: torch.Tensor) -> bool:
    N, Kd = weight.shape
    M = x.numel() // x.shape[-1]
    return (LN_EPILOGUE and not torch.is_grad_enabled() and x.is_cuda and x.dtype == torch.bfloat16 and weight.dtype == torch.bfloat16
            and x.is_contiguous() and N % 320 == 0 and Kd % 64 == 0 and M % 160 == 0 and (M // 160) * (N // 320) > _cus(x.device)
            and M * max(Kd, 320) * 2 < (1 << 31) and N * Kd * 2 < (1 << 31) and os.environ.get("FMC_G160_PERSIST", "1") != "0")


def linear_lnc(x: torch.Tensor, weight: torch.Tensor, bias, pend, geglu: bool = False) -> torch.Tensor:
    stats, gamma, beta, _ = pend
    wg, c, b = _ln_folded_weight(weight, bias, gamma, beta)
    _dev(x, wg, c, b, stats)
    N, Kd = weight.shape
    M, ldx = _rows2d(x)
    n_out = N // 2 if geglu else N
    out = torch.empty(*x.shape[:-1], n_out, dtype=x.dtype, device=x.device)
    ln_epilogue_calls["consumed"] += 1
    wt = _w_tilemajor(wg) if W_TILEMAJOR else wg
    _log_call("own_linear", (M, N, Kd, "lnc-geglu" if geglu else "lnc", 0), 2.0 * M * N * Kd)
    _lib.check(_lib.load().fmc_linear_bf16_lnc(x.data_ptr(), wt.data_ptr(), out.data_ptr(), M, N, Kd, ldx, n_out, int(geglu), stats.data_ptr(),
                                               c.data_ptr(), b.data_ptr(), int(W_TILEMAJOR), _stream()), "fmc_linear_bf16_lnc")
    return out


def linear_ln(x: torch.Tensor, weight: torch.Tensor, bias, residual, alpha: float, residual2, ln: LnSpec) -> torch.Tensor:
    _dev(x, weight, bias, residual, ln.gamma, ln.beta, ln.pe)
    N, Kd = weight.shape
    M, ldx = _rows2d(x)
    out = torch.empty(*x.shape[:-1], N, dtype=x.dtype, device=x.device)
    ldres = 0 if residual is None else _rows2d(residual)[1]
    ln_epilogue_calls["emitted"] += 1
    if ln.stats_only:
        stats = torch.empty(M, 2, dtype=torch.float32, device=x.device)
        ln_out = None
    else:
        stats, ln_out = None, torch.empty_like(out)
    wt = _w_tilemajor(weight) if W_TILEMAJOR else weight
    _log_call("own_linear", (M, N, Kd, "ln", (residual is not None) + (residual2 is not None)), 2.0 * M * N * Kd)
    _lib.check(_lib.load().fmc_linear_bf16_ln(x.data_ptr(), wt.data_ptr(), _p(bias), _p(residual), out.data_ptr(), M, N, Kd, ldx, ldres, N,
                                              float(alpha), _p(residual2), _p(ln_out), ln.gamma.data_ptr(), ln.beta.data_ptr(), float(ln.eps),
                                              _p(ln.pe), int(ln.pe_inner), int(ln.pe_frames), _p(stats), int(W_TILEMAJOR), _stream()),
               "fmc_linear_bf16_ln")
    out._fmc_ln = (stats, ln.key, True) if ln.stats_only else (ln_out, ln.key, False)
    return out


GN_FOLD = os.environ.get("FMC_GN_FOLD", "1") != "0"
GN_FOLD_MAX_BYTES = 8 << 20


def gn_fold_ok(x: torch.Tensor, gn_tag, groups: int, weight: torch.Tensor, ln: Optional[LnSpec]) -> bool:
    if not GN_FOLD or gn_tag is None or torch.is_grad_enabled() or x.ndim != 3 or weight.ndim != 2:
        return False
    n_img, hw, C = x.shape
    N = weight.shape[0]
    M = n_img * hw
    return (x.is_cuda and x.dtype == torch.bfloat16 and x.is_contiguous() and weight.dtype == torch.bfloat16 and weight.is_contiguous() and weight.shape[1] == C
            and groups == 32 and gn_tag[1] == C and gn_tag[0].shape[0] == n_img and gn_tag[0].shape[1] <= 64 and gn_tag[0].shape[2] == groups
            and hw % 160 == 0 and C % 64 == 0 and N % 320 == 0 and (M // 160) * (N // 320) >= _cus(x.device) and n_img * N * C * 2 <= GN_FOLD_MAX_BYTES
            and M * max(C, N) * 2 < (1 << 31) and (ln is None or (LN_EPILOGUE and ln.stats_only and N == 320))
            and os.environ.get("FMC_G160_PERSIST", "1") != "0")


def linear_gnfold(x: torch.Tensor, gn_tag, gamma: torch.Tensor, beta: torch.Tensor, groups: int, eps: float, weight: torch.Tensor, bias,
                  ln: Optional[LnSpec] = None) -> torch.Tensor:
    part = gn_tag[0]
    _dev(x, part, gamma, beta, weight, bias)
    n_img, hw, C = x.shape
    N = weight.shape[0]
    M = n_img * hw
    lib = _lib.load()
    w_img = torch.empty(n_img, N, C, dtype=torch.bfloat16, device=x.device)
    b_img = torch.empty(n_img, N, dtype=torch.float32, device=x.device)
    gn_epilogue_calls["consumed"] += 1
    _lib.check(lib.fmc_groupnorm_fold_linear(part.data_ptr(), int(part.shape[1]), gamma.data_ptr(), beta.data_ptr(), weight.data_ptr(), _p(bias),
                                             w_img.data_ptr(), b_img.data_ptr(), n_img, hw, C, int(groups), N, float(eps), int(W_TILEMAJOR), _stream()),
               "fmc_groupnorm_fold_linear")
    out = torch.empty(n_img, hw, N, dtype=x.dtype, device=x.device)
    stats = None
    if ln is not None:
        stats = torch.empty(M, 2, dtype=torch.float32, device=x.device)
        ln_epilogue_calls["emitted"] += 1
    _log_call("own_linear", (M, N, C, "gn-fold", 0), 2.0 * M * N * C)
    _lib.check(lib.fmc_linear_bf16_imgw(x.data_ptr(), w_img.data_ptr(), b_img.data_ptr(), out.data_ptr(), M, N, C, C, N, hw, _p(stats),
                                        float(ln.eps) if ln is not None else 0.0, int(W_TILEMAJOR), _stream()), "fmc_linear_bf16_imgw")
    if ln is not None:
        out._fmc_ln = (stats, ln.key, True)
    return out


FF_BLOCKED = os.environ.get("FMC_FF_BLOCKED", "1") != "0"


def ff_blocked_ok(x: torch.Tensor, w1_il160: Optional[torch.Tensor], w2: torch.Tensor, residual) -> bool:
    if not FF_BLOCKED or w1_il160 is None or torch.is_grad_enabled():
        return False
    N1, Kd = w1_il160.shape
    N2, Cff = w2.shape
    M = x.numel() // x.shape[-1]
    return (x.is_cuda and x.dtype == torch.bfloat16 and w1_il160.dtype == torch.bfloat16 and w2.dtype == torch.bfloat16 and x.is_contiguous()
            and w1_il160.is_contiguous() and w2.is_contiguous() and N1 == 2 * Cff and Cff % 160 == 0 and N2 % 320 == 0 and Kd % 64 == 0
            and M % 160 == 0 and M >= 16384 and (M // 160) * (N1 // 320) > _cus(x.device) and M * Cff * 2 < (1 << 31)
            and (residual is None or (residual.is_contiguous() and residual.dtype == x.dtype))
            and os.environ.get("FMC_G160_PERSIST", "1") != "0")


def geglu_linear_blocked(x: torch.Tensor, weight_il160: torch.Tensor, bias_il160) -> torch.Tensor:
    pend = getattr(x, "_fmc_pending_ln", None)
    N, Kd = weight_il160.shape
    M = x.numel() // Kd
    out = torch.empty(*x.shape[:-1], N // 2, dtype=x.dtype, device=x.device)
    if pend is not None:
        stats, gamma, beta, _ = pend
        wg, c, b = _ln_folded_weight(weight_il160, bias_il160, gamma, beta)
        _dev(x, wg, c, b, stats)
        ln_epilogue_calls["consumed"] += 1
        wt = _w_tilemajor(wg) if W_TILEMAJOR else wg
        args = (wt.data_ptr(), None, None, out.data_ptr(), M, N, Kd, 0, 1.0, 1, 0, 1, stats.data_ptr(), c.data_ptr(), b.data_ptr(), int(W_TILEMAJOR))
    else:
        _dev(x, weight_il160, bias_il160)
        wt = _w_tilemajor(weight_il160) if W_TILEMAJOR else weight_il160
        args = (wt.data_ptr(), _p(bias_il160), None, out.data_ptr(), M, N, Kd, 0, 1.0, 1, 0, 1, None, None, None, int(W_TILEMAJOR))
    _log_call("own_linear", (M, N, Kd, "geglu-blocked", 0), 2.0 * M * N * Kd)
    _lib.check(_lib.load().fmc_linear_bf16_ffblk(x.data_ptr(), *args, _stream()), "fmc_linear_bf16_ffblk")
    return out


def linear_from_blocked(xb: torch.Tensor, weight: torch.Tensor, bias, residual, alpha: float = 1.0, out: Optional[torch.Tensor] = None,
                        partial_tiles: bool = False) -> torch.Tensor:
    _dev(xb, weight, bias, residual, out)
    N, Kd = weight.shape
    M = xb.numel() // Kd
    if out is None:
        out = torch.empty(*xb.shape[:-1], N, dtype=xb.dtype, device=xb.device)
    assert out.is_contiguous() and out.numel() == M * N and out.dtype == xb.dtype
    wt = _w_tilemajor(weight) if W_TILEMAJOR else weight
    if partial_tiles:
        assert _blocked_storage_ok(xb, M, Kd), "linear_from_blocked: the tile-major operand does not own its padded storage"
        _log_call("own_linear", (M, N, Kd, "from-blocked-partial", int(residual is not None)), 2.0 * M * N * Kd)
        _lib.check(_lib.load().fmc_linear_bf16_ffblk_partial(xb.data_ptr(), wt.data_ptr(), _p(bias), _p(residual), out.data_ptr(), M, N, Kd,
                                                             0 if residual is None else N, float(alpha), int(W_TILEMAJOR), _stream()),
                   "fmc_linear_bf16_ffblk_partial")
        return out
    _log_call("own_linear", (M, N, Kd, "from-blocked", int(residual is not None)), 2.0 * M * N * Kd)
    _lib.check(_lib.load().fmc_linear_bf16_ffblk(xb.data_ptr(), wt.data_ptr(), _p(bias), _p(residual), out.data_ptr(), M, N, Kd,
                                                 0 if residual is None else N, float(alpha), 0, 1, 0, None, None, None, int(W_TILEMAJOR), _stream()),
               "fmc_linear_bf16_ffblk")
    return out


FF_TAIL = os.environ.get("FMC_FF_TAIL", "1") != "0"


def ff_tail_ok(h: torch.Tensor, w2: torch.Tensor, wp: torch.Tensor, tail_residual: Optional[torch.Tensor]) -> bool:
    C = h.shape[-1]
    M = h.numel() // C
    return (FF_TAIL and not torch.is_grad_enabled() and h.dtype == torch.bfloat16 and h.is_contiguous() and wp.dtype == torch.bfloat16 and w2.dtype == torch.bfloat16
            and wp.ndim == 2 and wp.shape[1] == w2.shape[0] == C and wp.shape[0] % 320 == 0 and C % 64 == 0 and w2.shape[1] % 64 == 0
            and M % 160 == 0 and (M // 160) * (wp.shape[0] // 320) >= _cus(h.device) and M * max(w2.shape[1], C) * 2 < (1 << 31)
            and tail_residual is not None and tail_residual.dtype == h.dtype and tail_residual.is_contiguous()
            and tail_residual.numel() == M * wp.shape[0] and os.environ.get("FMC_G160_PERSIST", "1") != "0")


def fold_ff_tail(w2: torch.Tensor, b2: Optional[torch.Tensor], wp: torch.Tensor, bp: Optional[torch.Tensor]):
    with torch.no_grad():
        wpf = wp.detach().float()
        wc = torch.cat([wpf @ w2.detach().float(), wpf], dim=1).to(torch.bfloat16).contiguous()
        bc = None
        if b2 is not None or bp is not None:
            bc = (wpf @ b2.detach().float()) if b2 is not None else torch.zeros(wp.shape[0], dtype=torch.float32, device=wp.device)
            if bp is not None:
                bc = bc + bp.detach().float()
            bc = bc.to(torch.bfloat16).contiguous()
    return wc, bc


def ff_tail(mid_blocked: torch.Tensor, h: torch.Tensor, w_cat: torch.Tensor, b_cat: Optional[torch.Tensor], tail_residual: torch.Tensor,
            gn_hw: int = 0, partial_tiles: bool = False) -> torch.Tensor:
    _dev(mid_blocked, h, w_cat, b_cat, tail_residual)
    N, Kd = w_cat.shape
    C = h.shape[-1]
    M = h.numel() // C
    assert mid_blocked.numel() == M * (Kd - C) and tail_residual.numel() == M * N
    out = torch.empty_like(tail_residual)
    if partial_tiles:
        assert _blocked_storage_ok(mid_blocked, M, Kd - C), "ff_tail: the tile-major operand does not own its padded storage"
        wt = _w_tilemajor(w_cat) if W_TILEMAJOR else w_cat
        _log_call("own_linear", (M, N, Kd, "ff-tail-partial", 1), 2.0 * M * N * Kd)
        _lib.check(_lib.load().fmc_linear_bf16_fftail_partial(mid_blocked.data_ptr(), h.data_ptr(), wt.data_ptr(), _p(b_cat), tail_residual.data_ptr(),
                                                              out.data_ptr(), M, N, Kd, Kd - C, C, N, None, 0, int(W_TILEMAJOR), _stream()),
                   "fmc_linear_bf16_fftail_partial")
        return out
    part = None
    if gn_hw and gn_emit_ok(M, N, Kd, gn_hw, h.dtype):
        part = torch.empty(M // gn_hw, gn_hw // 160, 32, 2, dtype=torch.float32, device=h.device)
        gn_epilogue_calls["emitted"] += 1
    wt = _w_tilemajor(w_cat) if W_TILEMAJOR else w_cat
    _log_call("own_linear", (M, N, Kd, "ff-tail", 1), 2.0 * M * N * Kd)
    _lib.check(_lib.load().fmc_linear_bf16_fftail(mid_blocked.data_ptr(), h.data_ptr(), wt.data_ptr(), _p(b_cat), tail_residual.data_ptr(), out.data_ptr(),
                                                  M, N, Kd, Kd - C, C, N, _p(part), int(gn_hw if part is not None else 0), int(W_TILEMAJOR), _stream()),
               "fmc_linear_bf16_fftail")
    if part is not None:
        out._fmc_gn = (part, N)
    return out


def linear_gn(x: torch.Tensor, weight: torch.Tensor, bias, residual, alpha: float, residual2, hw: int):
    _dev(x, weight, bias, residual)
    N, Kd = weight.shape
    M, ldx = _rows2d(x)
    out = torch.empty(*x.shape[:-1], N, dtype=x.dtype, device=x.device)
    part = torch.empty(M // hw, hw // 160, 32, 2, dtype=torch.float32, device=x.device)
    ldres = 0 if residual is None else _rows2d(residual)[1]
    gn_epilogue_calls["emitted"] += 1
    wt = _w_tilemajor(weight) if W_TILEMAJOR else weight
    _log_call("own_linear", (M, N, Kd, "gn", (residual is not None) + (residual2 is not None)), 2.0 * M * N * Kd)
    _lib.check(_lib.load().fmc_linear_bf16_gn(x.data_ptr(), wt.data_ptr(), _p(bias), _p(residual), out.data_ptr(), M, N, Kd, ldx, ldres, N,
                                              float(alpha), _p(residual2), part.data_ptr(), int(hw), int(W_TILEMAJOR), _stream()), "fmc_linear_bf16_gn")
    out._fmc_gn = (part, N)
    return out


def conv3x3_gn(x_nhwc: torch.Tensor, weight_cl: torch.Tensor, bias, temb, residual_nhwc, temb_div: int, upsample: bool, stride2: bool):
    n, h, w, cin = x_nhwc.shape
    if upsample:
        h, w = 2 * h, 2 * w
    if stride2:
        h, w = h // 2, w // 2
    cout = weight_cl.shape[0]
    out = torch.empty(n, h, w, cout, dtype=x_nhwc.dtype, device=x_nhwc.device)
    part = torch.empty(n, (h * w) // 160, 32, 2, dtype=torch.float32, device=x_nhwc.device)
    gn_epilogue_calls["emitted"] += 1
    wt = _w_tilemajor_conv(weight_cl) if W_TILEMAJOR else weight_cl
    _lib.check(_lib.load().fmc_conv3x3_bf16_gn(x_nhwc.data_ptr(), wt.data_ptr(), _p(bias), _p(temb), _p(residual_nhwc), out.data_ptr(),
                                               n, h, w, cin, cout, 0 if temb is None else temb.stride(0), int(temb_div),
                                               2 if stride2 else int(upsample), part.data_ptr(), int(W_TILEMAJOR), _stream()), "fmc_conv3x3_bf16_gn")
    return out, (part, cout)

# ... 473 lines not shown
_tune_log = {}
_calls = {}
AUTOTUNE = os.environ.get("FMC_AUTOTUNE", "1") != "0"
DETERMINISTIC = os.environ.get("FMC_DETERMINISTIC", "0") == "1"
_CACHE_ENV = os.environ.get("FMC_AUTOTUNE_CACHE", "")
_cache_state = {"loaded": False, "dirty": False, "meta": None}


def _cache_path():
    if _CACHE_ENV == "0":
        return None
    return _CACHE_ENV or os.path.join(os.path.dirname(_lib.LIB_PATH), "autotune_cache.json")


def _cache_meta():
    if _cache_state["meta"] is None:
        import hashlib
        with open(_lib.LIB_PATH, "rb") as f:
            sha = hashlib.sha256(f.read()).hexdigest()[:16]
        _cache_state["meta"] = {"lib_sha16": sha, "device": torch.cuda.get_device_name() if torch.cuda.is_available() else "cpu",
                                "arms": list(GEMM_TILES), "hipblaslt": vendor_version() if torch.cuda.is_available() else 0}
    return _cache_state["meta"]


DEFAULT_ARM_TABLE = os.path.join(os.path.dirname(os.path.abspath(__file__)), "autotune_default_mi355x.json")
stale_table_entries = [0]
autotune_sources = {"cache": 0, "defaults": 0}


def _load_table_file(path: str, strict_meta: bool) -> int:
    import ast
    import json
    if not path or not os.path.isfile(path):
        return 0
    try:
        with open(path) as f:
            blob = json.load(f)
        meta, mine = blob.get("meta") or {}, _cache_meta()
        if strict_meta and meta != mine:
            return 0
        if not strict_meta:
            arch = torch.cuda.get_device_properties(torch.cuda.current_device()).gcnArchName.split(":")[0]
            if meta.get("arch") != arch:
                return 0
        n = 0
        for k, v in blob["choices"].items():
            key = ast.literal_eval(k)
            if key[0] == "valgo" and meta.get("hipblaslt") != mine["hipblaslt"]:
                continue
            if key not in _choice:
                _choice[key] = int(v["arm"])
                _tune_log[key] = {int(a): ms for a, ms in v.get("ms", {}).items()}
                n += 1
        return n
    except Exception:
        return 0


def load_autotune_table(path: Optional[str] = None) -> int:
    _cache_state["loaded"] = True
    n = _load_table_file(path or _cache_path(), True)
    autotune_sources["cache"] += n
    if os.environ.get("FMC_AUTOTUNE_DEFAULTS", "1") != "0" and torch.cuda.is_available():
        d = _load_table_file(DEFAULT_ARM_TABLE, False)
        autotune_sources["defaults"] += d
        n += d
    return n


def save_autotune_table(path: Optional[str] = None) -> Optional[str]:
    import json
    path = path or _cache_path()
    if not path or not _choice:
        return None
    blob = {"meta": _cache_meta(),
            "choices": {repr(k): {"arm": v, "ms": _tune_log.get(k, {})} for k, v in _choice.items()}}
    tmp = f"{path}.{os.getpid()}.tmp"
    try:
        with open(tmp, "w") as f:
            json.dump(blob, f)
        os.replace(tmp, path)
    except OSError:
        return None
    _cache_state["dirty"] = False
    return path


def _save_at_exit():
    if _cache_state["dirty"] and os.environ.get("RANK", "0") == "0":
        save_autotune_table()


atexit.register(_save_at_exit)
GEMM_TILES = (1, 2, 3, 4, 5, 6, 7, 11,
              13,
              15,
              ARM_160B if W_TILEMAJOR else ARM_160,
              128 + 2, 128 + 3,
              128 + 13,
              256 + 13,
              384 + 13)
if os.environ.get("FMC_GEMM_ARMS"):
    GEMM_TILES = tuple(int(a) for a in os.environ["FMC_GEMM_ARMS"].split(","))


def autotune_report():
    return [(k, _choice[k], _tune_log.get(k, {}), _calls.get(k, 0)) for k in _choice]


_tune_stream = None
def _graph_ms(body, reps):
    g = torch.cuda.CUDAGraph()
    with torch.cuda.graph(g, stream=_tune_stream):
        for _ in range(reps):
            body()
    g.replay()
    _tune_stream.synchronize()
    ms = float("inf")
    for _ in range(3):
        e0, e1 = torch.cuda.Event(enable_timing=True), torch.cuda.Event(enable_timing=True)
        e0.record()
        g.replay()
        e1.record()
        _tune_stream.synchronize()
        ms = min(ms, e0.elapsed_time(e1) / reps)
    del g
    return ms


def _time_ms(fn, reps=8):
    global _tune_stream
    if _tune_stream is None:
        _tune_stream = torch.cuda.Stream()
    cur = torch.cuda.current_stream()
    _tune_stream.wait_stream(cur)
    with torch.cuda.stream(_tune_stream):
        fn()
        _tune_stream.synchronize()
        ms = _graph_ms(fn, reps)
    cur.wait_stream(_tune_stream)
    return ms


NO_VENDOR = os.environ.get("FMC_NO_VENDOR", "0") == "1"
dispatch_calls = {k: {"own": 0, "vendor": 0, "ineligible": 0} for k in ("linear", "geglu", "conv3x3")}
call_log = None


def _log_call(family: str, shape: tuple, flops: float) -> None:
    if call_log is not None:
        call_log.append((family, tuple(shape), float(flops)))


def _pick(key, hip_fn, lib_fn, static_hip: bool, extra_arms=(), k320: bool = False, own_only: bool = False) -> int:
    if not _cache_state["loaded"]:
        load_autotune_table()
    no_lib = (DETERMINISTIC and key[0] == "conv") or own_only or NO_VENDOR
    if no_lib:
        key = key + ("det",)
    use = _choice.get(key)
    _calls[key] = _calls.get(key, 0) + 1
    n320 = (key[5] if key[0] == "conv" else key[2]) % 320 == 0
    cands = tuple(t for t in GEMM_TILES + tuple(extra_arms)
                  if (t != 15 or k320)
                  and (not (ARM_160 <= t < ARM_160 + 5 or ARM_160B <= t < ARM_160B + 5 or t == ARM_256) or n320))
    if use is not None and not (use in cands or (use == 0 and not no_lib) or (use == -1 and key not in _tune_log)):
        _choice.pop(key, None)
        _tune_log.pop(key, None)
        stale_table_entries[0] += 1
        use = None
    if use is None:
        if not AUTOTUNE or torch.cuda.is_current_stream_capturing():
            return 0 if not (static_hip or no_lib) else -1
        times = ([] if no_lib else [(_time_ms(lib_fn), 0)]) + [(_time_ms(lambda t=t: hip_fn(t)), t) for t in cands]
        use = min(times)[1]
        _choice[key] = use
        _tune_log[key] = {arm: round(ms, 4) for ms, arm in times}
        _cache_state["dirty"] = True
    return use


def linear(x: torch.Tensor, weight: torch.Tensor, bias: Optional[torch.Tensor] = None,
           residual: Optional[torch.Tensor] = None, alpha: float = 1.0, x2: Optional[torch.Tensor] = None,
           residual2: Optional[torch.Tensor] = None, gn_hw: int = 0, ln: Optional["LnSpec"] = None,
           lazy_residual: bool = False) -> torch.Tensor:
    import torch.nn.functional as F
    pend = getattr(x, "_fmc_pending_ln", None)
    if pend is not None:
        if (x2 is None and residual is None and residual2 is None and alpha == 1.0 and not gn_hw and ln is None and weight.is_contiguous()
                and lnc_ok(x, weight)):
            dispatch_calls["linear"]["own"] += 1
            return linear_lnc(x, weight, bias, pend)
        x = resolve_pending_ln(x)

    def lib():
        xin = x if x2 is None else torch.cat([x, x2], dim=-1)
        if alpha == 1.0 and vendor_linear_ok(xin, weight, bias, residual):
            y = vendor_linear(xin, weight, bias, residual)
            return y if residual2 is None else y + residual2
        y = F.linear(xin, weight, bias)
        _log_call("vendor", (xin.numel() // xin.shape[-1], weight.shape[0], weight.shape[1], bias is not None, False), 2.0 * xin.numel() * weight.shape[0])
        if residual is not None:
            y = torch.add(residual, y, alpha=alpha)
            return y if residual2 is None else y + residual2
        return y if alpha == 1.0 else y * alpha

    N, Kd = weight.shape
    if (F32_GEMM and x.is_cuda and x.dtype == torch.float32 and weight.dtype == torch.float32 and Kd % 64 == 0 and N % 8 == 0
            and x.shape[-1] % 8 == 0 and (x.is_contiguous() or x.ndim == 2) and (x2 is None or x2.is_contiguous())
            and (residual is None or residual.dtype == torch.float32)):
        M = x.numel() // x.shape[-1]
        key = ("lin", M, N, Kd, bias is not None, (residual is not None) + (residual2 is not None), 0 if x2 is None else x.shape[-1])
        return linear_f32(x, weight, bias, residual, alpha, tile=_f32_arm(key, 0), x2=x2, residual2=residual2)
    ok = x.is_cuda and x.dtype == torch.bfloat16 and weight.dtype == torch.bfloat16 and Kd % 64 == 0 and N % 8 == 0
    if x2 is None:
        ok = ok and linear_supported(x, weight)
    else:
        ok = ok and x.shape[-1] % 64 == 0 and x2.dtype == x.dtype and x2.is_contiguous()
    if not ok or (x.ndim > 2 and not x.is_contiguous()):
        dispatch_calls["linear"]["ineligible"] += 1
        return lib()
    M = x.numel() // x.shape[-1]
    if ln is not None and x2 is None and not gn_hw and ln_emit_ok(x, weight, residual, residual2, ln):
        dispatch_calls["linear"]["own"] += 1
        return linear_ln(x, weight, bias, residual, alpha, residual2, ln)
    if (gn_hw and x2 is None and x.is_contiguous() and gn_emit_ok(M, N, Kd, gn_hw, x.dtype)
            and (residual is None or (residual.is_contiguous() and residual.dtype == x.dtype))
            and (residual2 is None or residual2.is_contiguous())):
        dispatch_calls["linear"]["own"] += 1
        return linear_gn(x, weight, bias, residual, alpha, residual2, gn_hw)
    key = ("lin", M, N, Kd, bias is not None, (residual is not None) + (residual2 is not None),
           0 if x2 is None else x.shape[-1])
    hip = lambda tile: (linear4_bf16(x, weight, bias, residual, alpha, residual2) if tile == ARM_G4
                        else linear_bf16(x, weight, bias, residual, alpha, tile=tile, x2=x2, residual2=residual2))
    small = (ARM_SMALLM, ARM_SMALLM + 2) if (M <= 2560 and x2 is None and residual2 is None) else ()
    t160 = ((M + 159) // 160) * ((N + 159) // 160)
    if (LINEAR4 and x2 is None and weight.is_contiguous() and 48 <= t160 <= 640 and Kd >= 320
            and _lib.load().fmc_linear4_supported(M, N, Kd, _rows2d(x)[1])
            and (residual is None or _rows2d(residual)[1] % 8 == 0)
            and (residual2 is None or (residual is not None and _rows2d(residual2)[1] == _rows2d(residual)[1]))):
        small = small + (ARM_G4,)
    use = _pick(key, hip, lib, Kd <= 640 and N <= 1024 and M >= 16384, split_arms(M, N, Kd) + small,
                k320=(Kd == 320 and N % 320 == 0 and M % 64 == 0 and x2 is None and residual2 is None))
    if (use == 0 and lazy_residual and LAZY_RESIDUAL and residual is not None and residual2 is None and alpha == 1.0 and x2 is None
            and N in (320, 640, 1280) and residual.is_contiguous() and not torch.is_grad_enabled()
            and not vendor_linear_ok(x, weight, bias, residual)):
        dispatch_calls["linear"]["vendor"] += 1
        y = F.linear(x, weight, bias)
        y._fmc_pending_add = residual
        return y
    dispatch_calls["linear"]["vendor" if use == 0 else "own"] += 1
    return lib() if use == 0 else hip(max(use, 0))


def geglu_linear(x: torch.Tensor, weight: torch.Tensor, bias, weight_il: torch.Tensor, bias_il, weight_il160=None,
                 bias_il160=None) -> torch.Tensor:
    import torch.nn.functional as F
    pend = getattr(x, "_fmc_pending_ln", None)
    if pend is not None:
        if weight_il160 is not None and weight_il160.is_contiguous() and lnc_ok(x, weight_il160):
            return linear_lnc(x, weight_il160, bias_il160, pend, geglu=True)
        x = resolve_pending_ln(x)
    lib = lambda: geglu(F.linear(x, weight, bias))
    if (F32_GEMM and x.is_cuda and x.dtype == torch.float32 and weight_il.dtype == torch.float32 and weight_il.shape[0] % 64 == 0
            and weight_il.shape[1] % 64 == 0 and x.is_contiguous()):
        N, Kd = weight.shape
        arm = _f32_arm(("geglu", x.numel() // Kd, N, Kd), 0)
        if arm in (ARM_160, ARM_160B) and weight_il160 is not None:
            return linear_f32(x, weight_il160, bias_il160, geglu=True, tile=ARM_160)
        return linear_f32(x, weight_il, bias_il, geglu=True, tile=0 if arm in (ARM_160, ARM_160B) else arm)
    if not linear_supported(x, weight_il) or weight_il.shape[0] % 64 or (x.ndim > 2 and not x.is_contiguous()):
        dispatch_calls["geglu"]["ineligible"] += 1
        return lib()
    N, Kd = weight.shape
    M = x.numel() // Kd
    has160 = weight_il160 is not None and N % 320 == 0

    def hip(tile):
        if tile in (ARM_160, ARM_256, ARM_160B):
            return linear_bf16(x, weight_il160, bias_il160, geglu=True, tile=tile) if has160 else linear_bf16(x, weight_il, bias_il, geglu=True, tile=13)
        return linear_bf16(x, weight_il, bias_il, geglu=True, tile=tile)
    use = _pick(("geglu", M, N, Kd), hip, lib, M >= 65536)
    dispatch_calls["geglu"]["vendor" if use == 0 else "own"] += 1
    return lib() if use == 0 else hip(max(use, 0))


def conv3x3(x_nchw: torch.Tensor, weight_cl: torch.Tensor, bias, temb=None, residual_nchw=None, stride=(1, 1),
            padding=(1, 1), temb_div: int = 1, upsample: bool = False, emit_gn: bool = False, own_only: bool = False, shortcut=None) -> torch.Tensor:
    import torch.nn.functional as F

    if shortcut is not None:
        n, cin, h, w = x_nchw.shape
        cout = weight_cl.shape[0]
        xs, xs2, w_sc, b_sc = shortcut
        assert temb is None and residual_nchw is None and not upsample and tuple(stride) == (1, 1) and tuple(padding) == (1, 1)
        if not shortcut_fold_ok(x_nchw, weight_cl, xs, xs2):
            raise RuntimeError("conv3x3: no kernel takes this shape with the shortcut in the reduction")
        want = bool(emit_gn and GN_EPILOGUE and cout % 64 == 0 and 160 % (cout // 32) == 0)
        dispatch_calls["conv3x3"]["own"] += 1
        cs1 = xs.shape[1]
        y = conv3x3_halo(x_nchw.permute(0, 2, 3, 1), weight_cl, bias, emit_gn=want,
                         shortcut=(xs.permute(0, 2, 3, 1), None if xs2 is None else xs2.permute(0, 2, 3, 1), w_sc, b_sc),
                         partial_tiles=_shortcut_fold_partial(n, h, w, cin, cout, cs1 + (xs2.shape[1] if xs2 is not None else 0), cs1))
        return _gn_tagged(y, want, cout)

    def lib():
        xin = F.interpolate(x_nchw, scale_factor=2.0, mode="nearest") if upsample else x_nchw
        y = F.conv2d(xin, weight_cl, bias, stride, padding)
        if temb is not None:
            y = y + (temb if temb_div == 1 else temb.repeat_interleave(temb_div, dim=0))[:, :, None, None]
        if residual_nchw is not None:
            y = y + residual_nchw
        return y

    if (F32_GEMM and x_nchw.is_cuda and x_nchw.dtype == torch.float32 and weight_cl.dtype == torch.float32
            and tuple(weight_cl.shape[2:]) == (3, 3) and tuple(padding) == (1, 1) and weight_cl.shape[1] % 64 == 0
            and weight_cl.shape[0] % 8 == 0 and (tuple(stride) == (1, 1) or (tuple(stride) == (2, 2) and not upsample
                                                                           and x_nchw.shape[-1] % 2 == 0 and x_nchw.shape[-2] % 2 == 0))):
        n, cin, h, w = x_nchw.shape
        x = x_nchw.permute(0, 2, 3, 1)
        r = None if residual_nchw is None else residual_nchw.permute(0, 2, 3, 1)
        if x.is_contiguous() and (r is None or r.is_contiguous()) and (temb is None or temb.stride(1) == 1):
            s2 = tuple(stride) == (2, 2)
            ho, wo = (2 * h, 2 * w) if upsample else ((h // 2, w // 2) if s2 else (h, w))
            key = ("conv", n, ho, wo, cin, weight_cl.shape[0], temb is not None, r is not None, upsample, s2)
            return conv3x3_f32(x, weight_cl, bias, temb, r, tile=_f32_arm(key, 0), temb_div=temb_div, upsample=upsample,
                               stride2=s2).permute(0, 3, 1, 2)
    if not conv3x3_supported(x_nchw, weight_cl, stride, padding):
        dispatch_calls["conv3x3"]["ineligible"] += 1
        return lib()
    n, cin, h, w = x_nchw.shape
    cout = weight_cl.shape[0]
    x = x_nchw.permute(0, 2, 3, 1)
    r = None if residual_nchw is None else residual_nchw.permute(0, 2, 3, 1)
    if not x.is_contiguous() or (r is not None and not r.is_contiguous()):
        dispatch_calls["conv3x3"]["ineligible"] += 1
        return lib()
    if upsample:
        h, w = 2 * h, 2 * w
    stride2 = tuple(stride) == (2, 2)
    if stride2:
        h, w = h // 2, w // 2
    if upsample and temb is None and r is None and not torch.is_grad_enabled() and x.dtype == torch.bfloat16 and weight_cl.dtype == torch.bfloat16:
# ... 797 lines not shown
```

Before: 39.34 steps/s.

## Add K=320 GEMM forms for LayerNorm-consumer and GroupNorm-folded per-image weights

Extends the K=320 register-resident-weight GEMM kernel with fused variants. One applies a folded LayerNorm epilogue using per-row stats. The other uses per-image GroupNorm-folded weights and biases, optionally emitting LayerNorm row statistics. The variants use a persistent walker schedule with contiguous tile ranges per block, and are chosen by autotuning against the existing 160-row ring kernel. This lets small-shape or non-ring-eligible LN/GN-fused linears take the fused path instead of falling back to an unfused or ring path, at the cost of reloading weights whenever a walker crosses an image boundary.

```diff
diff --git a/include/fmc_hip.h b/include/fmc_hip.h
--- a/include/fmc_hip.h
+++ b/include/fmc_hip.h
@@ -102,6 +102,11 @@
                               void* w_out, float* bias_out, int n_img, int HW, int C, int G, int N, float eps, int w_tilemajor, void* stream);
 int fmc_linear_bf16_imgw(const void* x, const void* w_img, const float* bias_img, void* out, int64_t M, int N, int K, int64_t ldx, int64_t ldo,
                          int img_rows, float* ln_stats, float ln_eps, int w_tilemajor, void* stream);
+int fmc_linear_bf16_lnc_k320(const void* x, const void* w_gamma, void* out, int64_t M, int N, int K, int64_t ldx, int64_t ldo,
+                             const float* ln_stats, const float* ln_c, const float* ln_bias, void* stream);
+int fmc_linear_bf16_imgw_k320(const void* x, const void* w_img, const float* bias_img, void* out, int64_t M, int N, int K, int64_t ldx, int64_t ldo,
+                              int img_rows, float* ln_stats, float ln_eps, void* stream);
+int fmc_linear_k320_form_walkers(int64_t M, int N);
 int fmc_linear_bf16_fftail(const void* x_blocked, const void* x2, const void* w, const void* bias, const void* residual, void* out, int64_t M,
                            int N, int K, int k_split, int64_t ldx2, int64_t ldres, float* gn_partials, int gn_hw, int w_tilemajor, void* stream);
 int fmc_linear_bf16_ffblk_partial(const void* x_blocked, const void* w, const void* bias, const void* residual, void* out, int64_t M, int N, int K,
diff --git a/synfmc_amd/_lib.py b/synfmc_amd/_lib.py
--- a/synfmc_amd/_lib.py
+++ b/synfmc_amd/_lib.py
@@ -60,6 +60,10 @@
                                           c_float, c_int, c_void_p]),
     "fmc_linear_bf16_imgw": (c_int, [c_void_p, c_void_p, c_void_p, c_void_p, c_int64, c_int, c_int, c_int64, c_int64, c_int, c_void_p, c_float, c_int,
                                      c_void_p]),
+    "fmc_linear_bf16_lnc_k320": (c_int, [c_void_p, c_void_p, c_void_p, c_int64, c_int, c_int, c_int64, c_int64, c_void_p, c_void_p, c_void_p, c_void_p]),
+    "fmc_linear_bf16_imgw_k320": (c_int, [c_void_p, c_void_p, c_void_p, c_void_p, c_int64, c_int, c_int, c_int64, c_int64, c_int, c_void_p, c_float,
+                                          c_void_p]),
+    "fmc_linear_k320_form_walkers": (c_int, [c_int64, c_int]),
     "fmc_linear_bf16_fftail": (c_int, [c_void_p, c_void_p, c_void_p, c_void_p, c_void_p, c_void_p, c_int64, c_int, c_int, c_int, c_int64, c_int64,
                                        c_void_p, c_int, c_int, c_void_p]),
     "fmc_conv3x3_bf16_gn": (c_int, [c_void_p, c_void_p, c_void_p, c_void_p, c_void_p, c_void_p, c_int, c_int, c_int, c_int, c_int,
diff --git a/synfmc_amd/csrc/gemm_conv.hip b/synfmc_amd/csrc/gemm_conv.hip
--- a/synfmc_amd/csrc/gemm_conv.hip
+++ b/synfmc_amd/csrc/gemm_conv.hip
@@ -2272,8 +2272,14 @@
     return (size_t)2 * 32 * MI * K320_K * 2 + (size_t)k320_stage_chunks<MI, NI>() * 16 + 160 * NI * sizeof(float);
 }
 
-template <int MI, int NI, bool HAS_RES>
+constexpr int K320_XS_BYTES = 2 * 1024 + 320 * (int)sizeof(float);
+template <int MI, int NI> constexpr size_t k320_xs_off() { return (k320_lds<MI, NI>() + 1023) / 1024 * 1024; }
+
+template <int MI, int NI, bool HAS_RES, int LN = 0, int LNC = 0, int IMG = 0>
 __global__ __launch_bounds__(320, (MI * NI == 1 ? 3 : (MI * NI == 2 ? 2 : 1))) void gemm_k320_kernel(const GemmParams P) {
+    constexpr bool FORM = LN || LNC || IMG;
+    static_assert(!FORM || (MI == 2 && NI == 2 && !HAS_RES), "fused forms: the 64 x 320 geometry, no residual");
+    static_assert((LN == 0 || LN == 2) && !(LNC && (LN || IMG)), "forms: LayerNorm consumer | per-image weights, the latter with or without row statistics");
     constexpr int K = K320_K, KS = K / 16, BM = 32 * MI, BN = 160 * NI, OP = BN + 8, CPR = K / 8, OCPR = OP / 8, WC = 32 * NI;
     constexpr int A_ELEMS = BM * K, A_PIECES = BM * CPR / 64, ST_PIECES = k320_stage_chunks<MI, NI>() / 64;
     constexpr int A_PPW = (A_PIECES + 4) / 5, ST_PPW = (ST_PIECES + 4) / 5;
@@ -2281,23 +2287,66 @@
     bf16_t* Abuf = reinterpret_cast<bf16_t*>(smem_raw);
     bf16_t* Os = Abuf + 2 * A_ELEMS;
     float* bias_s = reinterpret_cast<float*>(Os + k320_stage_chunks<MI, NI>() * 8);
+    float* stat_s = reinterpret_cast<float*>(smem_raw + k320_xs_off<MI, NI>());
+    float* c_s = stat_s + 512;
     const int tid = threadIdx.x, lane = tid & 63, wave = __builtin_amdgcn_readfirstlane(tid >> 6);
     const int l31 = lane & 31, half = lane >> 5;
-    const int n0 = blockIdx.y * BN;
-    const int ntiles = (int)(P.M / BM);
+    int f_n0 = 0, f_t = 0, f_tend = 0;
+    if constexpr (FORM) {
+        const int nb = P.N / BN, g = (int)gridDim.x, nwalk = g / nb, id = (int)blockIdx.x, nt = (int)(P.M / BM);
+        int cb, w;
+        if (g % (8 * nb) == 0) {
+            const int j = id >> 3;
+            cb = j % nb;
+            w = (id & 7) * (nwalk >> 3) + j / nb;
+        } else {
+            cb = id % nb;
+            w = id / nb;
+        }
+        const int per = nt / nwalk, rem = nt - per * nwalk;
+        f_n0 = cb * BN;
+        f_t = w * per + (w < rem ? w : rem);
+        f_tend = f_t + per + (w < rem ? 1 : 0);
+    }
+    const int n0 = FORM ? f_n0 : blockIdx.y * BN;
+    const int ntiles = FORM ? f_tend : (int)(P.M / BM);
+    const unsigned tstep = FORM ? 1u : gridDim.x;
 
     bf16x8 wf[KS][NI];
-#pragma unroll
-    for (int ni = 0; ni < NI; ++ni) {
-        const bf16_t* wrow = P.w + (int64_t)(n0 + wave * WC + ni * 32 + l31) * K + half * 8;
-#pragma unroll
-        for (int ks = 0; ks < KS; ++ks) {
-            union { bf16x8 v; u32x4 u; } t;
-            t.u = *reinterpret_cast<const u32x4*>(wrow + ks * 16);
-            wf[ks][ni] = t.v;
-        }
-    }
-    for (int i = tid; i < BN; i += 320) bias_s[i] = P.bias ? bf2f(P.bias[n0 + i]) : 0.f;
+    int img = 0;
+    auto load_w_img = [&](int l31w, int halfw) {
+#pragma unroll
+        for (int ni = 0; ni < NI; ++ni) {
+            const bf16_t* wrow = P.w + (int64_t)img * P.w_img_stride + (int64_t)(n0 + wave * WC + ni * 32 + l31w) * K + halfw * 8;
+#pragma unroll
+            for (int ks = 0; ks < KS; ++ks) {
+                union { bf16x8 v; u32x4 u; } t;
+                t.u = *reinterpret_cast<const u32x4*>(wrow + ks * 16);
+                wf[ks][ni] = t.v;
+            }
+        }
+    };
+    if constexpr (IMG) {
+        img = f_t < f_tend ? f_t * BM / P.img_rows : 0;
+        load_w_img(l31, half);
+        for (int i = tid; i < BN; i += 320) bias_s[i] = P.bias_img[(int64_t)img * P.N + n0 + i];
+    } else {
+#pragma unroll
+        for (int ni = 0; ni < NI; ++ni) {
+            const bf16_t* wrow = P.w + (int64_t)(n0 + wave * WC + ni * 32 + l31) * K + half * 8;
+#pragma unroll
+            for (int ks = 0; ks < KS; ++ks) {
+                union { bf16x8 v; u32x4 u; } t;
+                t.u = *reinterpret_cast<const u32x4*>(wrow + ks * 16);
+                wf[ks][ni] = t.v;
+            }
+        }
+        if constexpr (LNC) {
+            for (int i = tid; i < BN; i += 320) { bias_s[i] = P.lnc_bias[n0 + i]; c_s[i] = P.lnc_c[n0 + i]; }
+        } else {
+            for (int i = tid; i < BN; i += 320) bias_s[i] = P.bias ? bf2f(P.bias[n0 + i]) : 0.f;
+        }
+    }
 
     const __amdgpu_buffer_rsrc_t rsA = __builtin_amdgcn_make_buffer_rsrc((void*)P.a, 0, (int)(((P.M - 1) * P.lda + K) * 2), 0x00020000);
     const __amdgpu_buffer_rsrc_t rsR = __builtin_amdgcn_make_buffer_rsrc((void*)(HAS_RES ? P.res + n0 : P.a), 0,
@@ -2327,28 +2376,46 @@
         for (int i = 0; i < ST_PPW; ++i)
             if (wave + 5 * i < ST_PIECES) dma(rsR, r_vo(wave + 5 * i), soff, Os + (wave + 5 * i) * 512);
     };
+    const __amdgpu_buffer_rsrc_t rsS = __builtin_amdgcn_make_buffer_rsrc((void*)(LNC ? (const void*)P.lnc_stats : (const void*)P.a), 0, LNC ? (int)(P.M * 8) : 0, 0x00020000);
+    auto load_stats = [&](int tile, int buf) {
+        if (wave == 4) dma(rsS, lane_v < BM / 2 ? (unsigned)(lane_v * 16) : OOB, tile * BM * 8, reinterpret_cast<bf16_t*>(stat_s + buf * 256));
+    };
 
     const int sw = (l31 >> 1) & 7, x6 = sw & 6, b0 = half ^ (sw & 1);
     int dsel[4];
 #pragma unroll
     for (int m = 0; m < 4; ++m) dsel[m] = l31 * K + (x6 - 2 * (x6 & (2 * m)) + b0) * 8;
 
-    int t = blockIdx.x;
+    int t = FORM ? f_t : blockIdx.x;
     if (t < ntiles) load_a(t, 0);
-    if (t + (int)gridDim.x < ntiles) load_a(t + gridDim.x, 1);
+    if (t + (int)tstep < ntiles) load_a(t + tstep, 1);
     if (HAS_RES && t < ntiles) load_res(t);
+    if constexpr (LNC) {
+        if (t < ntiles) load_stats(t, 0);
+        if (t + 1 < ntiles) load_stats(t + 1, 1);
+    }
     asm volatile("s_waitcnt vmcnt(0)" ::: "memory");
     __syncthreads();
 
-    for (int it = 0; t < ntiles; t += gridDim.x, ++it) {
+    for (int it = 0; t < ntiles; t += tstep, ++it) {
         const bf16_t* As = Abuf + (it & 1) * A_ELEMS;
         asm volatile("" : "+v"(lane_v), "+v"(tid_v));
+        if constexpr (IMG) {
+            const int ti = t * BM / P.img_rows;
+            if (ti != img) {
+                img = ti;
+                load_w_img(lane_v & 31, lane_v >> 5);
+                for (int i = tid_v; i < BN; i += 320) bias_s[i] = P.bias_img[(int64_t)img * P.N + n0 + i];
+                asm volatile("s_waitcnt vmcnt(0) lgkmcnt(0)\n\ts_barrier" ::: "memory");
+            }
+        }
         f32x16 acc[NI][MI];
 #pragma unroll
         for (int a = 0; a < NI; ++a)
 #pragma unroll
             for (int g = 0; g < 4; ++g) {
-                const f32x4 bv = *reinterpret_cast<const f32x4*>(bias_s + wave * WC + a * 32 + 8 * g + 4 * half);
+                f32x4 bv = {0.f, 0.f, 0.f, 0.f};
+                if constexpr (!LNC) bv = *reinterpret_cast<const f32x4*>(bias_s + wave * WC + a * 32 + 8 * g + 4 * half);
 #pragma unroll
                 for (int b = 0; b < MI; ++b)
 #pragma unroll
@@ -2378,7 +2445,7 @@
         asm volatile("s_waitcnt vmcnt(0) lgkmcnt(0)\n\ts_barrier" ::: "memory");
         asm volatile("" : "+v"(lane_v), "+v"(tid_v));
         const int l31_e = lane_v & 31, half_e = (lane_v >> 5) & 1;
-        if (t + 2 * (int)gridDim.x < ntiles) load_a(t + 2 * gridDim.x, it & 1);
+        if (t + 2 * (int)tstep < ntiles) load_a(t + 2 * tstep, it & 1);
 
 #pragma unroll
         for (int ni = 0; ni < NI; ++ni)
@@ -2395,6 +2462,13 @@
                     float o[4];
 #pragma unroll
                     for (int j = 0; j < 4; ++j) o[j] = P.alpha * acc[ni][mi][4 * g + j];
+                    if constexpr (LNC) {
+                        const f32x2_t st = *reinterpret_cast<const f32x2_t*>(stat_s + (it & 1) * 256 + (mi * 32 + l31_e) * 2);
+                        const f32x4 c4 = *reinterpret_cast<const f32x4*>(c_s + wave * WC + ni * 32 + 8 * g + 4 * half_e);
+                        const f32x4 b4 = *reinterpret_cast<const f32x4*>(bias_s + wave * WC + ni * 32 + 8 * g + 4 * half_e);
+#pragma unroll
+                        for (int j = 0; j < 4; ++j) o[j] = st[1] * (acc[ni][mi][4 * g + j] - st[0] * c4[j]) + b4[j];
+                    }
                     if (HAS_RES) {
                         o[0] += __uint_as_float(rw[g][0] << 16); o[1] += __uint_as_float(rw[g][0] & 0xffff0000u);
                         o[2] += __uint_as_float(rw[g][1] << 16); o[3] += __uint_as_float(rw[g][1] & 0xffff0000u);
@@ -2410,9 +2484,37 @@
                 *reinterpret_cast<u32x4*>(og + (int64_t)r * P.ldo + ch * 8) = *reinterpret_cast<const u32x4*>(Os + r * OP + ch * 8);
             }
         }
+        if constexpr (LN == 2) {
+            if (tid_v < 4 * BM) {
+                const int r = tid_v >> 2, q = tid_v & 3;
+                float s1 = 0.f, s2 = 0.f;
+#pragma unroll
+                for (int i = 0; i < 10; ++i) {
+                    const u32x4 x4 = *reinterpret_cast<const u32x4*>(Os + r * OP + (q + 4 * i) * 8);
+#pragma unroll
+                    for (int j = 0; j < 4; ++j) s1 += __uint_as_float(x4[j] << 16) + __uint_as_float(x4[j] & 0xffff0000u);
+                }
+                s1 += __shfl_xor(s1, 1); s1 += __shfl_xor(s1, 2);
+                const float mean = s1 * (1.f / 320.f);
+#pragma unroll
+                for (int i = 0; i < 10; ++i) {
+                    const u32x4 x4 = *reinterpret_cast<const u32x4*>(Os + r * OP + (q + 4 * i) * 8);
+#pragma unroll
+                    for (int j = 0; j < 4; ++j) {
+                        const float lo = __uint_as_float(x4[j] << 16) - mean, hi = __uint_as_float(x4[j] & 0xffff0000u) - mean;
+                        s2 += lo * lo + hi * hi;
+                    }
+                }
+                s2 += __shfl_xor(s2, 1); s2 += __shfl_xor(s2, 2);
+                if (q == 0) *reinterpret_cast<f32x2_t*>(P.ln_stats + ((int64_t)t * BM + r) * 2) = f32x2_t{mean, rsqrtf(s2 * (1.f / 320.f) + P.ln_eps)};
+            }
+        }
+        if constexpr (LNC) {
+            if (t + 2 < ntiles) load_stats(t + 2, it & 1);
+        }
         if (HAS_RES) {
             asm volatile("s_waitcnt lgkmcnt(0)\n\ts_barrier" ::: "memory");
-            if (t + (int)gridDim.x < ntiles) load_res(t + gridDim.x);
+            if (t + (int)tstep < ntiles) load_res(t + tstep);
         }
     }
 }
@@ -2421,12 +2523,23 @@
     static const int v = fmc_env_int("FMC_K320_CFG", 22);
     return v;
 }
+inline bool gemm_k320_is_form(const GemmParams& P) { return P.lnc_stats || P.bias_img || P.ln_stats || P.ln_out || P.gn_part; }
 bool gemm_k320_ok(const GemmParams& P) {
     const int bn = (gemm_k320_cfg() % 10 == 1) ? 160 : 320;
-    return !P.f32io && P.hw <= 1 && P.K == K320_K && P.N % bn == 0 && P.M % 64 == 0 && !P.a2 && !P.res2 && P.split_k == 1 && !P.sk && !P.temb &&
-           ((P.M - 1) * P.lda + P.K) * 2 < ((int64_t)1 << 31) && (!P.res || ((P.M - 1) * P.ldres + P.N) * 2 < ((int64_t)1 << 31));
-}
-
+    if (!(!P.f32io && P.hw <= 1 && P.K == K320_K && P.N % bn == 0 && P.M % 64 == 0 && !P.a2 && !P.res2 && P.split_k == 1 && !P.sk && !P.temb &&
+          ((P.M - 1) * P.lda + P.K) * 2 < ((int64_t)1 << 31) && (!P.res || ((P.M - 1) * P.ldres + P.N) * 2 < ((int64_t)1 << 31))))
+        return false;
+    if (!gemm_k320_is_form(P)) return true;
+    return P.N % 320 == 0 && !P.ln_out && !P.gn_part && !P.res && !P.bias && !P.a_blocked && !P.out_blocked && !P.w_blocked &&
+           (P.lnc_stats ? !P.bias_img && !P.ln_stats && P.M * 8 < ((int64_t)1 << 31)
+                        : P.bias_img && P.img_rows >= 64 && P.img_rows % 64 == 0 && P.M % P.img_rows == 0 && (!P.ln_stats || P.N == 320));
+}
+int gemm_k320_form_walkers(int64_t M, int N) {
+    const int nb = N / 320, tiles = (int)(M / 64);
+    int w = (fmc_cu_count() / (8 * nb)) * 8;
+    if (w < 8) w = fmc_cu_count() / nb > 0 ? fmc_cu_count() / nb : 1;
+    return tiles < w ? tiles : w;
+}
 template <int MI, int NI>
 void launch_gemm_k320_c(GemmParams& P, hipStream_t st) {
     const size_t lds = k320_lds<MI, NI>();
@@ -2436,7 +2549,16 @@
     if (P.res) fmc_launch<gemm_k320_kernel<MI, NI, true>>(grid, dim3(320), lds, st, P);
     else fmc_launch<gemm_k320_kernel<MI, NI, false>>(grid, dim3(320), lds, st, P);
 }
+void launch_gemm_k320_form(GemmParams& P, hipStream_t st) {
+    const size_t lds = k320_xs_off<2, 2>() + K320_XS_BYTES;
+    static_assert(k320_xs_off<2, 2>() + K320_XS_BYTES <= 160 * 1024, "the forms' statistics and column constants fit behind the plain layout");
+    const dim3 grid((unsigned)(gemm_k320_form_walkers(P.M, P.N) * (P.N / 320))), block(320);
+    if (P.lnc_stats) fmc_launch<gemm_k320_kernel<2, 2, false, 0, 1, 0>>(grid, block, lds, st, P);
+    else if (P.ln_stats) fmc_launch<gemm_k320_kernel<2, 2, false, 2, 0, 1>>(grid, block, lds, st, P);
+    else fmc_launch<gemm_k320_kernel<2, 2, false, 0, 0, 1>>(grid, block, lds, st, P);
+}
 void launch_gemm_k320(GemmParams& P, hipStream_t st) {
+    if (gemm_k320_is_form(P)) { launch_gemm_k320_form(P, st); return; }
     switch (gemm_k320_cfg()) {
         case 11: launch_gemm_k320_c<1, 1>(P, st); break;
         case 21: launch_gemm_k320_c<2, 1>(P, st); break;
@@ -2632,10 +2754,11 @@
     P.gn_part = (float*)gn_partials; P.gn_hw = gn_hw;
     if (lnc_stats) {
         const int cus = fmc_cu_count() & ~7;
-        if (f32io || tile != 16 || split_k != 1 || gn_partials || ln_out || ln_stats || x2 || bias || residual || residual2 || alpha != 1.f || N % 320 ||
+        if (tile != 15 &&
+            (f32io || tile != 16 || split_k != 1 || gn_partials || ln_out || ln_stats || x2 || bias || residual || residual2 || alpha != 1.f || N % 320 ||
             M % 160 || (M / 160) * (N / 320) <= cus || cus < 8 || !lnc_c || !lnc_bias || !fmc_aligned16(lnc_c) || !fmc_aligned16(lnc_bias) ||
             ((M - 1) * ldx + K) * 2 >= ((int64_t)1 << 31) || (int64_t)N * K * 2 >= ((int64_t)1 << 31) ||
-            g160_persist() == 0)
+            g160_persist() == 0))
             FMC_FAIL(FMC_E_SHAPE, "linear_bf16_lnc: tile 16's persistent form only (bf16, N %% 320 == 0, M %% 160 == 0, more tiles than CUs, no bf16 bias / "
                                   "residual, alpha 1)");
     }
@@ -2655,10 +2778,11 @@
     P.bias_img = nullptr; P.w_img_stride = 0; P.img_rows = 0;
     if (bias_img) {
         const int cus = fmc_cu_count() & ~7;
-        if (f32io || epilogue != 0 || tile != 16 || split_k != 1 || gn_partials || x2 || bias || residual || residual2 || alpha != 1.f || ln_out || lnc_stats ||
+        if (tile != 15 &&
+            (f32io || epilogue != 0 || tile != 16 || split_k != 1 || gn_partials || x2 || bias || residual || residual2 || alpha != 1.f || ln_out || lnc_stats ||
             a_blocked || out_blocked || N % 320 || M % 160 || (M / 160) * (N / 320) < cus || cus < 8 || img_rows < 160 || img_rows % 160 || M % img_rows ||
             ((uintptr_t)bias_img & 15) || ((M - 1) * ldx + K) * 2 >= ((int64_t)1 << 31) || (M / img_rows) * (int64_t)N * K * 2 >= ((int64_t)1 << 31) ||
-            g160_persist() == 0)
+            g160_persist() == 0))
             FMC_FAIL(FMC_E_SHAPE, "linear_bf16_imgw: tile 16's persistent form only (bf16, N %% 320 == 0, M %% 160 == 0, at least as many tiles as CUs, images of a multiple "
                                   "of 160 rows, no bf16 bias / residual, all weights < 2 GiB)");
         P.bias_img = bias_img; P.w_img_stride = (int64_t)N * K; P.img_rows = img_rows;
@@ -2666,9 +2790,10 @@
     if (ln_out || ln_stats) {
         const int cus = fmc_cu_count() & ~7;
         if ((ln_out != nullptr) == (ln_stats != nullptr)) FMC_FAIL(FMC_E_NULL, "linear_bf16_ln: exactly one of ln_out / ln_stats");
-        if (f32io || epilogue != 0 || tile != 16 || split_k != 1 || gn_partials || x2 || N != 320 || M % 160 || (bias_img ? M / 160 < cus : M / 160 <= cus) || cus < 8 ||
+        if (tile != 15 &&
+            (f32io || epilogue != 0 || tile != 16 || split_k != 1 || gn_partials || x2 || N != 320 || M % 160 || (bias_img ? M / 160 < cus : M / 160 <= cus) || cus < 8 ||
             (ln_out && (!ln_gamma || !ln_beta || !fmc_aligned16(ln_out))) || (ln_stats && ((uintptr_t)ln_stats & 7)) || (ln_pe && (ln_pe_inner <= 0 || ln_pe_inner % 160 || ln_pe_frames <= 0)) ||
-            ((M - 1) * ldx + K) * 2 >= ((int64_t)1 << 31) || g160_persist() == 0)
+            ((M - 1) * ldx + K) * 2 >= ((int64_t)1 << 31) || g160_persist() == 0))
             FMC_FAIL(FMC_E_SHAPE, "linear_bf16_ln: the LayerNorm output comes out of tile 16's persistent form only (bf16, N == 320, M %% 160 == 0, "
                                   "M / 160 > CUs, plain epilogue, positional-encoding frames of a multiple of 160 rows)");
     }
@@ -2687,6 +2812,14 @@
         P.w_blocked = 1;
     }
     if (int rc = set_split_k(P, split_k, workspace, workspace_bytes, epilogue == 0, "linear_bf16")) return rc;
+    if (tile == 15 && gemm_k320_is_form(P)) {
+        if (epilogue != 0 || alpha != 1.f || w_tilemajor || gemm_k320_cfg() != 22 || gemm_geometry_override() != 0 || !gemm_k320_ok(P) ||
+            (lnc_stats && (!lnc_c || !lnc_bias || !fmc_aligned16(lnc_stats) || !fmc_aligned16(lnc_c) || !fmc_aligned16(lnc_bias))) ||
+            (bias_img && ((uintptr_t)bias_img & 15)) || (ln_stats && ((uintptr_t)ln_stats & 7)))
+            FMC_FAIL(FMC_E_SHAPE, "linear_bf16: tile 15 takes the LayerNorm-consumer form and per-image weights (with or without row statistics, N == 320) "
+                                  "only: bf16, K == 320, N %% 320 == 0, M %% 64 == 0, images of a multiple of 64 rows, row-major weights, no bf16 bias / residual, "
+                                  "alpha 1 (M=%lld N=%d K=%d)", (long long)M, N, K);
+    }
     if (epilogue == 0) launch_gemm<0, 0>(P, tile, st); else launch_gemm<0, 1>(P, tile, st);
     FMC_CHECK_LAUNCH("fmc_linear_bf16");
     return 0;
@@ -2740,6 +2873,22 @@
     return linear_impl(x, w_img, nullptr, nullptr, out, M, N, K, ldx, 0, ldo, 1.f, 0, 16, 1, nullptr, 0, nullptr, 0, 0, nullptr, stream, 0,
                        nullptr, 0, nullptr, nullptr, nullptr, ln_eps, nullptr, 1, 1, ln_stats, nullptr, nullptr, nullptr, 0, 0, w_tilemajor, bias_img, img_rows);
 }
+
+extern "C" int fmc_linear_bf16_lnc_k320(const void* x, const void* w_gamma, void* out, int64_t M, int N, int K, int64_t ldx, int64_t ldo,
+                                        const float* ln_stats, const float* ln_c, const float* ln_bias, void* stream) {
+    if (!ln_stats || !ln_c || !ln_bias) FMC_FAIL(FMC_E_NULL, "linear_bf16_lnc_k320: NULL ln_stats / ln_c / ln_bias");
+    return linear_impl(x, w_gamma, nullptr, nullptr, out, M, N, K, ldx, 0, ldo, 1.f, 0, 15, 1, nullptr, 0, nullptr, 0, 0, nullptr, stream, 0,
+                       nullptr, 0, nullptr, nullptr, nullptr, 0.f, nullptr, 1, 1, nullptr, ln_stats, ln_c, ln_bias, 0, 0, 0);
+}
+
+extern "C" int fmc_linear_bf16_imgw_k320(const void* x, const void* w_img, const float* bias_img, void* out, int64_t M, int N, int K, int64_t ldx, int64_t ldo,
+                                         int img_rows, float* ln_stats, float ln_eps, void* stream) {
+    if (!bias_img) FMC_FAIL(FMC_E_NULL, "linear_bf16_imgw_k320: NULL bias_img");
+    return linear_impl(x, w_img, nullptr, nullptr, out, M, N, K, ldx, 0, ldo, 1.f, 0, 15, 1, nullptr, 0, nullptr, 0, 0, nullptr, stream, 0,
+                       nullptr, 0, nullptr, nullptr, nullptr, ln_eps, nullptr, 1, 1, ln_stats, nullptr, nullptr, nullptr, 0, 0, 0, bias_img, img_rows);
+}
+
+extern "C" int fmc_linear_k320_form_walkers(int64_t M, int N) { return (M < 64 || N < 320 || N % 320) ? 0 : gemm_k320_form_walkers(M, N); }
 
 extern "C" int fmc_linear_bf16_fftail(const void* x_blocked, const void* x2, const void* w, const void* bias, const void* residual, void* out, int64_t M,
                                       int N, int K, int k_split, int64_t ldx2, int64_t ldres, float* gn_partials, int gn_hw, int w_tilemajor, void* stream) {
diff --git a/synfmc_amd/hip_ops.py b/synfmc_amd/hip_ops.py
--- a/synfmc_amd/hip_ops.py
+++ b/synfmc_amd/hip_ops.py
@@ -1651,6 +1651,31 @@
             and M * max(Kd, 320) * 2 < (1 << 31) and N * Kd * 2 < (1 << 31) and os.environ.get("FMC_G160_PERSIST", "1") != "0")
 
 
+K320_FORMS = int(os.environ.get("FMC_K320_FORMS", "1"))
+k320_form_calls = {"lnc": 0, "imgw": 0}
+
+
+def _k320_rows_ok(x: torch.Tensor) -> bool:
+    return x.is_contiguous() or (x.ndim == 2 and x.stride(1) == 1 and x.stride(0) % 8 == 0 and x.data_ptr() % 16 == 0)
+
+
+def lnc_k320_ok(x: torch.Tensor, weight: torch.Tensor) -> bool:
+    N, Kd = weight.shape
+    M = x.numel() // x.shape[-1]
+    return (K320_FORMS != 0 and LN_EPILOGUE and not torch.is_grad_enabled() and x.is_cuda and x.dtype == torch.bfloat16 and weight.dtype == torch.bfloat16
+            and _k320_rows_ok(x) and Kd == 320 and N % 320 == 0 and M % 64 == 0 and M > 0 and (M - 1) * _rows2d(x)[1] * 2 + 640 < (1 << 31)
+            and M * N * 2 < (1 << 31))
+
+
+def _k320_form_arm(kind: str, M: int, N: int, Kd: int, ring_ok: bool, launch) -> bool:
+    if not ring_ok or K320_FORMS == 2:
+        return True
+    ring = ARM_160B if W_TILEMAJOR else ARM_160
+    if 15 not in GEMM_TILES or ring not in GEMM_TILES:
+        return False
+    return _pick(("lin", M, N, Kd, kind), launch, None, True, k320=True, own_only=True, only=(15, ring)) == 15
+
+
 def linear_lnc(x: torch.Tensor, weight: torch.Tensor, bias, pend, geglu: bool = False) -> torch.Tensor:
     stats, gamma, beta, _ = pend
     wg, c, b = _ln_folded_weight(weight, bias, gamma, beta)
@@ -1660,11 +1685,22 @@
     n_out = N // 2 if geglu else N
     out = torch.empty(*x.shape[:-1], n_out, dtype=x.dtype, device=x.device)
     ln_epilogue_calls["consumed"] += 1
-    wt = _w_tilemajor(wg) if W_TILEMAJOR else wg
+    lib = _lib.load()
+
+    def launch(arm):
+        if arm == 15:
+            _lib.check(lib.fmc_linear_bf16_lnc_k320(x.data_ptr(), wg.data_ptr(), out.data_ptr(), M, N, Kd, ldx, n_out, stats.data_ptr(), c.data_ptr(),
+                                                    b.data_ptr(), _stream()), "fmc_linear_bf16_lnc_k320")
+        else:
+            wt = _w_tilemajor(wg) if W_TILEMAJOR else wg
+            _lib.check(lib.fmc_linear_bf16_lnc(x.data_ptr(), wt.data_ptr(), out.data_ptr(), M, N, Kd, ldx, n_out, int(geglu), stats.data_ptr(),
+                                               c.data_ptr(), b.data_ptr(), int(W_TILEMAJOR), _stream()), "fmc_linear_bf16_lnc")
+        return out
+    arm = 15 if (not geglu and lnc_k320_ok(x, weight) and stats.is_contiguous()
+                 and _k320_form_arm("lnc", M, N, Kd, lnc_ok(x, weight), launch)) else 16
+    k320_form_calls["lnc"] += arm == 15
     _log_call("own_linear", (M, N, Kd, "lnc-geglu" if geglu else "lnc", 0), 2.0 * M * N * Kd)
-    _lib.check(_lib.load().fmc_linear_bf16_lnc(x.data_ptr(), wt.data_ptr(), out.data_ptr(), M, N, Kd, ldx, n_out, int(geglu), stats.data_ptr(),
-                                               c.data_ptr(), b.data_ptr(), int(W_TILEMAJOR), _stream()), "fmc_linear_bf16_lnc")
-    return out
+    return launch(arm)
 
 
 def linear_ln(x: torch.Tensor, weight: torch.Tensor, bias, residual, alpha: float, residual2, ln: LnSpec) -> torch.Tensor:
@@ -1701,9 +1737,17 @@
     M = n_img * hw
     return (x.is_cuda and x.dtype == torch.bfloat16 and x.is_contiguous() and weight.dtype == torch.bfloat16 and weight.is_contiguous() and weight.shape[1] == C
             and groups == 32 and gn_tag[1] == C and gn_tag[0].shape[0] == n_img and gn_tag[0].shape[1] <= 64 and gn_tag[0].shape[2] == groups
-            and hw % 160 == 0 and C % 64 == 0 and N % 320 == 0 and (M // 160) * (N // 320) >= _cus(x.device) and n_img * N * C * 2 <= GN_FOLD_MAX_BYTES
+            and C % 64 == 0 and N % 320 == 0 and n_img * N * C * 2 <= GN_FOLD_MAX_BYTES
             and M * max(C, N) * 2 < (1 << 31) and (ln is None or (LN_EPILOGUE and ln.stats_only and N == 320))
-            and os.environ.get("FMC_G160_PERSIST", "1") != "0")
+            and _gn_fold_ring_ok(n_img, hw, C, N, x.device))
+
+
+def _gn_fold_ring_ok(n_img: int, hw: int, C: int, N: int, device) -> bool:
+    return hw % 160 == 0 and (n_img * hw // 160) * (N // 320) >= _cus(device) and os.environ.get("FMC_G160_PERSIST", "1") != "0"
+
+
+def _gn_fold_k320_ok(hw: int, C: int) -> bool:
+    return K320_FORMS != 0 and C == 320 and hw % 64 == 0
 
 
 def linear_gnfold(x: torch.Tensor, gn_tag, gamma: torch.Tensor, beta: torch.Tensor, groups: int, eps: float, weight: torch.Tensor, bias,
@@ -1717,17 +1761,29 @@
     w_img = torch.empty(n_img, N, C, dtype=torch.bfloat16, device=x.device)
     b_img = torch.empty(n_img, N, dtype=torch.float32, device=x.device)
     gn_epilogue_calls["consumed"] += 1
-    _lib.check(lib.fmc_groupnorm_fold_linear(part.data_ptr(), int(part.shape[1]), gamma.data_ptr(), beta.data_ptr(), weight.data_ptr(), _p(bias),
-                                             w_img.data_ptr(), b_img.data_ptr(), n_img, hw, C, int(groups), N, float(eps), int(W_TILEMAJOR), _stream()),
-               "fmc_groupnorm_fold_linear")
     out = torch.empty(n_img, hw, N, dtype=x.dtype, device=x.device)
     stats = None
     if ln is not None:
         stats = torch.empty(M, 2, dtype=torch.float32, device=x.device)
         ln_epilogue_calls["emitted"] += 1
+
+    def launch(arm):
+        wtm = int(W_TILEMAJOR and arm != 15)
+        _lib.check(lib.fmc_groupnorm_fold_linear(part.data_ptr(), int(part.shape[1]), gamma.data_ptr(), beta.data_ptr(), weight.data_ptr(), _p(bias),
+                                                 w_img.data_ptr(), b_img.data_ptr(), n_img, hw, C, int(groups), N, float(eps), wtm, _stream()),
+                   "fmc_groupnorm_fold_linear")
+        if arm == 15:
+            _lib.check(lib.fmc_linear_bf16_imgw_k320(x.data_ptr(), w_img.data_ptr(), b_img.data_ptr(), out.data_ptr(), M, N, C, C, N, hw, _p(stats),
+                                                     float(ln.eps) if ln is not None else 0.0, _stream()), "fmc_linear_bf16_imgw_k320")
+        else:
+            _lib.check(lib.fmc_linear_bf16_imgw(x.data_ptr(), w_img.data_ptr(), b_img.data_ptr(), out.data_ptr(), M, N, C, C, N, hw, _p(stats),
+                                                float(ln.eps) if ln is not None else 0.0, wtm, _stream()), "fmc_linear_bf16_imgw")
+        return out
+    arm = 15 if (_gn_fold_k320_ok(hw, C) and (ln is None or N == 320)
+                 and _k320_form_arm(f"imgw-ln:{hw}" if ln is not None else f"imgw:{hw}", M, N, C, _gn_fold_ring_ok(n_img, hw, C, N, x.device), launch)) else 16
+    k320_form_calls["imgw"] += arm == 15
     _log_call("own_linear", (M, N, C, "gn-fold", 0), 2.0 * M * N * C)
-    _lib.check(lib.fmc_linear_bf16_imgw(x.data_ptr(), w_img.data_ptr(), b_img.data_ptr(), out.data_ptr(), M, N, C, C, N, hw, _p(stats),
-                                        float(ln.eps) if ln is not None else 0.0, int(W_TILEMAJOR), _stream()), "fmc_linear_bf16_imgw")
+    launch(arm)
     if ln is not None:
         out._fmc_ln = (stats, ln.key, True)
     return out
@@ -2507,7 +2563,7 @@
         call_log.append((family, tuple(shape), float(flops)))
 
 
-def _pick(key, hip_fn, lib_fn, static_hip: bool, extra_arms=(), k320: bool = False, own_only: bool = False) -> int:
+def _pick(key, hip_fn, lib_fn, static_hip: bool, extra_arms=(), k320: bool = False, own_only: bool = False, only=None) -> int:
     if not _cache_state["loaded"]:
         load_autotune_table()
     no_lib = (DETERMINISTIC and key[0] == "conv") or own_only or NO_VENDOR
@@ -2518,7 +2574,8 @@
     n320 = (key[5] if key[0] == "conv" else key[2]) % 320 == 0
     cands = tuple(t for t in GEMM_TILES + tuple(extra_arms)
                   if (t != 15 or k320)
-                  and (not (ARM_160 <= t < ARM_160 + 5 or ARM_160B <= t < ARM_160B + 5 or t == ARM_256) or n320))
+                  and (not (ARM_160 <= t < ARM_160 + 5 or ARM_160B <= t < ARM_160B + 5 or t == ARM_256) or n320)
+                  and (only is None or t in only))
     if use is not None and not (use in cands or (use == 0 and not no_lib) or (use == -1 and key not in _tune_log)):
         _choice.pop(key, None)
         _tune_log.pop(key, None)
@@ -2543,7 +2600,7 @@
     pend = getattr(x, "_fmc_pending_ln", None)
     if pend is not None:
         if (x2 is None and residual is None and residual2 is None and alpha == 1.0 and not gn_hw and ln is None and weight.is_contiguous()
-                and lnc_ok(x, weight)):
+                and (lnc_ok(x, weight) or lnc_k320_ok(x, weight))):
             dispatch_calls["linear"]["own"] += 1
             return linear_lnc(x, weight, bias, pend)
         x = resolve_pending_ln(x)
```

Measured after the change: 39.39 steps/s (median of 6 runs). About the same (+0.1%).
